# ml4ai/mliis

Hardware: AMD Instinct MI355X
Metric: inner-loop images/sec (EfficientLab-6-3, 224x224, 5-shot) (higher is better)
Workload: dtype f32 (the long-K decoder convs and their filter gradients with every operand split exactly into three bf16 terms on the matrix cores, 6 term products, f32 accumulate: fp32-equivalent products; everything else the fp32 instruction)

## Files before the change

mliis_amd/csrc/dwmarch.hip:

```cpp
#include "bn_fold.hpp"
#include "common.hpp"

namespace mliis {

constexpr int kDwmStoreAux = 2;
typedef unsigned dwm_u32x4 __attribute__((ext_vector_type(4)));
constexpr unsigned kDwmOob = 0xFFFFFFF0u;

__device__ __forceinline__ __amdgpu_buffer_rsrc_t dwm_rsrc(const void* p) {
  const unsigned long long u = (unsigned long long)p;
  const unsigned lo = __builtin_amdgcn_readfirstlane((unsigned)u), hi = __builtin_amdgcn_readfirstlane((unsigned)(u >> 32));
  return __builtin_amdgcn_make_buffer_rsrc((void*)(((unsigned long long)hi << 32) | lo), 0, 0x80000000u, 0x00020000);
}

typedef unsigned dwm_u32x2 __attribute__((ext_vector_type(2)));
template <typename T = float>
__device__ __forceinline__ float4 dwm_load(__amdgpu_buffer_rsrc_t r, int off, bool ok) {
  if constexpr (sizeof(T) == 4) {
    const dwm_u32x4 u = __builtin_amdgcn_raw_buffer_load_b128(r, ok ? off : (int)kDwmOob, 0, 0);
    return make_float4(__uint_as_float(u.x), __uint_as_float(u.y), __uint_as_float(u.z), __uint_as_float(u.w));
  } else {
    const dwm_u32x2 u = __builtin_amdgcn_raw_buffer_load_b64(r, ok ? off : (int)kDwmOob, 0, 0);
    return unpack_bf16x4(make_uint2(u.x, u.y));
  }
}

template <typename T = float>
__device__ __forceinline__ void dwm_store(__amdgpu_buffer_rsrc_t r, int off, bool ok, const float4 v) {
  if constexpr (sizeof(T) == 2) {
    const uint2 pk = pack_bf16x4(v);
    dwm_u32x2 u2;
    u2.x = pk.x; u2.y = pk.y;
    __builtin_amdgcn_raw_buffer_store_b64(u2, r, ok ? off : (int)kDwmOob, 0, kDwmStoreAux);
    return;
  }
  dwm_u32x4 u;
  u.x = __float_as_uint(v.x); u.y = __float_as_uint(v.y); u.z = __float_as_uint(v.z); u.w = __float_as_uint(v.w);
  __builtin_amdgcn_raw_buffer_store_b128(u, r, ok ? off : (int)kDwmOob, 0, kDwmStoreAux);
}
__device__ __forceinline__ float4 f4sel(bool ok, const float4 v) { return ok ? v : make_float4(0.f, 0.f, 0.f, 0.f); }
template <typename T> __device__ __forceinline__ float4 dwm_stored(const float4 v) { return stored_value(static_cast<const T*>(nullptr), v); }

template <int K, int S>
struct MarchCfg {
  static constexpr int TS = S == 1 ? 4 : 2;
  static constexpr int BW = 7 * TS;
  static constexpr int SPR = BW / TS;
  static constexpr int RS = 4;
  static constexpr int IBW = (BW - 1) * S + K;
  static constexpr int IBWP = (IBW + 1) & ~1;
  static constexpr int WIN = (RS - 1) * S + K;
  static constexpr int NEW = RS * S;
  static constexpr int NR = WIN + NEW;
  static constexpr int WW = (TS - 1) * S + K;
  static_assert(IBW <= 32, "one pixel lane per ring column");
  static_assert(WIN <= 2 * NEW, "head batch + batch 0 cover the window of step 0");
};

struct DwmBn {
  BnFold f;
  const float* gamma;
  const float* beta;
};

struct DwmDyBn {
  const float* z;
  const float *mean, *rstd, *gamma, *beta;
  const float *gate, *chan_add;
  const float* stage1;
  int nimg;
  double inv_rows;
  float *dgamma, *dbeta;
};
struct DwmDyQuad {
  float4 sc, sh, gt, ca, k1, k0;
};
__device__ __forceinline__ DwmDyQuad dwm_dybn_setup(const DwmDyBn& d, int C, int c0, int q, bool cok, int n, bool lead) {
  const int c = cok ? c0 + q * 4 : 0;
  const float4 m = ld4(d.mean + c), rs = ld4(d.rstd + c), ga = ld4(d.gamma + c), be = ld4(d.beta + c);
  DwmDyQuad k;
  k.gt = ld4(d.gate + (long long)n * C + c);
  k.ca = ld4(d.chan_add + (long long)n * C + c);
  double s1[4] = {0, 0, 0, 0}, s2[4] = {0, 0, 0, 0};
  for (int i0 = 0; i0 < d.nimg; i0 += 8) {
    float4 u[8], v[8];
#pragma unroll
    for (int j = 0; j < 8; ++j) {
      const int i = i0 + j < d.nimg ? i0 + j : d.nimg - 1;
      u[j] = ld4(d.stage1 + ((long long)i * 2 + 0) * C + c);
      v[j] = ld4(d.stage1 + ((long long)i * 2 + 1) * C + c);
    }
#pragma unroll
    for (int j = 0; j < 8; ++j)
      if (i0 + j < d.nimg) {
        s1[0] += u[j].x; s1[1] += u[j].y; s1[2] += u[j].z; s1[3] += u[j].w;
        s2[0] += v[j].x; s2[1] += v[j].y; s2[2] += v[j].z; s2[3] += v[j].w;
      }
  }
  if (lead && cok && (threadIdx.x >> 3) == 0) {
    st4(d.dbeta + c, make_float4((float)s1[0], (float)s1[1], (float)s1[2], (float)s1[3]));
    st4(d.dgamma + c, make_float4((float)s2[0], (float)s2[1], (float)s2[2], (float)s2[3]));
  }
  const float4 a = make_float4((float)(s1[0] * d.inv_rows), (float)(s1[1] * d.inv_rows), (float)(s1[2] * d.inv_rows), (float)(s1[3] * d.inv_rows));
  const float4 b = make_float4((float)(s2[0] * d.inv_rows), (float)(s2[1] * d.inv_rows), (float)(s2[2] * d.inv_rows), (float)(s2[3] * d.inv_rows));
  k.sc = f4mul(ga, rs);
  k.sh = make_float4(fmaf(-m.x, k.sc.x, be.x), fmaf(-m.y, k.sc.y, be.y), fmaf(-m.z, k.sc.z, be.z), fmaf(-m.w, k.sc.w, be.w));
  k.k1 = make_float4(-k.sc.x * b.x * rs.x, -k.sc.y * b.y * rs.y, -k.sc.z * b.z * rs.z, -k.sc.w * b.w * rs.w);
  k.k0 = make_float4(-k.sc.x * a.x - k.k1.x * m.x, -k.sc.y * a.y - k.k1.y * m.y, -k.sc.z * a.z - k.k1.z * m.z, -k.sc.w * a.w - k.k1.w * m.w);
  return k;
}
__device__ __forceinline__ float dwm_dz1(float da2, float z, float sc, float sh, float gt, float ca, float k1, float k0) {
  const float u = fmaf(z, sc, sh);
  const float sg = sigmoid_f(u);
  const float g = fmaf(da2, gt, ca) * (sg * (1.0f + u * (1.0f - sg)));
  return fmaf(sc, g, fmaf(z, k1, k0));
}
__device__ __forceinline__ float4 dwm_dz1(const float4 da2, const float4 z, const DwmDyQuad& k) {
  return make_float4(dwm_dz1(da2.x, z.x, k.sc.x, k.sh.x, k.gt.x, k.ca.x, k.k1.x, k.k0.x), dwm_dz1(da2.y, z.y, k.sc.y, k.sh.y, k.gt.y, k.ca.y, k.k1.y, k.k0.y),
                     dwm_dz1(da2.z, z.z, k.sc.z, k.sh.z, k.gt.z, k.ca.z, k.k1.z, k.k0.z), dwm_dz1(da2.w, z.w, k.sc.w, k.sh.w, k.gt.w, k.ca.w, k.k1.w, k.k0.w));
}

template <int NEW, bool TWO>
struct DwmBatch {
  float4 a[NEW];
  float4 b[TWO ? NEW : 1];
};

struct DwmArgs {
  const float* x;
  const float* w;
  float* y;
  int Hi, Wi, Ho, Wo;
  int C, pt, pl;
  int bands, bw, chunks, rpc;
  float* stats_part;
  DwmBn bn;
  DwmDyBn dyb;
  const float* z;
  float* dw_part;
};

struct DwmQuad {
  float4 sc, sh, m, rs;
};

__device__ __forceinline__ float4 dwm_act(const float4 z, const DwmQuad& k) {
  float4 u = make_float4(fmaf(z.x, k.sc.x, k.sh.x), fmaf(z.y, k.sc.y, k.sh.y), fmaf(z.z, k.sc.z, k.sh.z), fmaf(z.w, k.sc.w, k.sh.w));
  return make_float4(swish_f(u.x), swish_f(u.y), swish_f(u.z), swish_f(u.w));
}

constexpr int kDwmFoldBatch = 8;
template <bool FOLD>
struct DwmBnState {
  float4 g, b, m, rs;
  FoldAcc acc;
  float4 u[FOLD ? kDwmFoldBatch : 1], v[FOLD ? kDwmFoldBatch : 1];
  int k;
};
template <bool FOLD>
__device__ __forceinline__ void dwm_bn_begin(const DwmBn& bn, int C, int c0, int q, bool cok, DwmBnState<FOLD>& st) {
  const int c = cok ? c0 + q * 4 : 0;
  st.g = ld4(bn.gamma + c);
  st.b = ld4(bn.beta + c);
  if (FOLD && bn.f.nblk > 0) {
    const int bl = threadIdx.x >> 3;
    st.k = bl;
    for (; st.k + 32 * kDwmFoldBatch < bn.f.nblk; st.k += 32 * kDwmFoldBatch) {
      fold_issue<FOLD ? kDwmFoldBatch : 1>(bn.f.part, bn.f.nblk, C, c, st.k, bl, st.u, st.v);
      if (cok) fold_add<FOLD ? kDwmFoldBatch : 1>(st.acc, bn.f.nblk, st.k, st.u, st.v);
    }
    fold_issue<FOLD ? kDwmFoldBatch : 1>(bn.f.part, bn.f.nblk, C, c, st.k, st.k < bn.f.nblk ? st.k : 0, st.u, st.v);
  } else {
    st.m = ld4(bn.f.mean + c);
    st.rs = ld4(bn.f.rstd + c);
  }
}
template <bool FOLD>
__device__ __forceinline__ DwmQuad dwm_bn_end(const DwmBn& bn, int C, int c0, int q, bool cok, bool lead, double* smd, float* s_mr ,
                                              DwmBnState<FOLD>& st) {
  const int t = threadIdx.x;
  DwmQuad k;
  if (FOLD && bn.f.nblk > 0) {
    if (cok) fold_add<FOLD ? kDwmFoldBatch : 1>(st.acc, bn.f.nblk, st.k, st.u, st.v);
    double s, ss;
    fold_finish(st.acc, smd, s, ss);
    if (t < 32) {
      const double m = s * bn.f.inv_n;
      double var = ss * bn.f.inv_n - m * m;
      if (var < 0.0) var = 0.0;
      const float mf = (float)m, rf = (float)(1.0 / sqrt(var + (double)bn.f.eps));
      s_mr[t] = mf;
      s_mr[32 + t] = rf;
      const int cc = c0 + t;
      if (lead && cc < C) {
        bn.f.mean[cc] = mf;
        bn.f.rstd[cc] = rf;
        if (bn.f.moving_mean != nullptr) {
          const float mm = bn.f.moving_mean[cc], mv = bn.f.moving_var[cc];
          bn.f.moving_mean[cc] = mm - (mm - mf) * bn.f.one_minus_momentum;
          bn.f.moving_var[cc] = mv - (mv - (float)(var * (double)bn.f.ema_var_factor)) * bn.f.one_minus_momentum;
        }
      }
    }
    __syncthreads();
    k.m = ld4(s_mr + q * 4);
    k.rs = ld4(s_mr + 32 + q * 4);
    __syncthreads();
  } else {
    k.m = st.m;
    k.rs = st.rs;
  }
  k.sc = f4mul(st.g, k.rs);
  k.sh = make_float4(fmaf(-k.m.x, k.sc.x, st.b.x), fmaf(-k.m.y, k.sc.y, st.b.y), fmaf(-k.m.z, k.sc.z, st.b.z), fmaf(-k.m.w, k.sc.w, st.b.w));
  return k;
}

__device__ __forceinline__ void dwm_emit_pair(const float4 s1, const float4 s2, float4* buf, float* __restrict__ part, unsigned blk, int C,
                                              int c0) {
  const int t = threadIdx.x;
  buf[t] = s1;
  buf[256 + t] = s2;
  __syncthreads();
  float4 v = f4zero();
  if (t < 64) {
    const int qq = t & 7, g = (t >> 3) & 3, vv = t >> 5;
#pragma unroll
    for (int i = 0; i < 8; ++i) v = f4add(v, buf[vv * 256 + (g * 8 + i) * 8 + qq]);
  }
  __syncthreads();
  if (t < 64) buf[t] = v;
  __syncthreads();
  if (t < 16) {
    const int qq = t & 7, vv = t >> 3;
    const int cc = c0 + qq * 4;
    const float4* b4 = buf + vv * 32 + qq;
    if (cc < C) st4(part + ((long long)blk * 2 + vv) * C + cc, f4add(f4add(b4[0], b4[8]), f4add(b4[16], b4[24])));
  }
}

template <int K, int S, bool PRE, bool BWD, bool DYBN = false, typename TA = float, typename TB = float>
__global__ __launch_bounds__(256, BWD ? 1 : 2) void dwm_conv_k(const DwmArgs a) {
  constexpr int EA = (int)sizeof(TA), EB = (int)sizeof(TB);
  static_assert(!DYBN || BWD, "DYBN is a backward mode");
  typedef MarchCfg<K, S> G;
  constexpr int TS = G::TS, SPR = G::SPR, RS = G::RS, IBW = G::IBW, IBWP = G::IBWP, WIN = G::WIN, NEW = G::NEW, NR = G::NR, WW = G::WW;
  static_assert(!BWD || S == 1, "the stride-2 backward is dwm_bwd_s2_k");
  constexpr int kRingF4 = (NR * IBWP + 1) * 8;
  constexpr int kTrash = NR * IBWP * 8;
  constexpr int kScratchF4 = BWD ? (K * K * 4 * 8) : 0;
  constexpr int kSharedF4 = kRingF4 > kScratchF4 ? kRingF4 : kScratchF4;
  static_assert(kSharedF4 * 16 >= 2 * 32 * 32 * 8, "the statistics fold borrows the ring");
  __shared__ float4 ring[kSharedF4];
  __shared__ float4 wl[K * K * 8];
  __shared__ __attribute__((aligned(16))) float s_mr[64];

  const int t = threadIdx.x, q = t & 7, p = t >> 3;
  const unsigned bx = xcd_remap(blockIdx.x, gridDim.x);
  const int chunk = (int)(bx % (unsigned)a.chunks);
  const unsigned r_ = bx / (unsigned)a.chunks;
  const int band = (int)(r_ % (unsigned)a.bands), n = (int)(r_ / (unsigned)a.bands);
  const int c0 = blockIdx.y * 32, c = c0 + q * 4;
  const bool cok = c < a.C;
  const int Hi = a.Hi, Wi = a.Wi, Ho = a.Ho, Wo = a.Wo, C = a.C;
  const int oy0 = chunk * a.rpc;
  const int oy1 = oy0 + a.rpc < Ho ? oy0 + a.rpc : Ho;
  const int ox0 = band * a.bw;
  const int bwa = a.bw < Wo - ox0 ? a.bw : Wo - ox0;
  const int iy0 = oy0 * S - a.pt, ix0 = ox0 * S - a.pl;
  const int ibw = (bwa - 1) * S + K;
  const int rows_needed = (oy1 - oy0 - 1) * S + K;
  const int nsteps = (oy1 - oy0 + RS - 1) / RS;
  const __amdgpu_buffer_rsrc_t rX = dwm_rsrc(a.x);
  const __amdgpu_buffer_rsrc_t rZ = dwm_rsrc((BWD ? a.z : a.x));
  const __amdgpu_buffer_rsrc_t rY = dwm_rsrc(a.y);

  const bool colok = cok && p < ibw && (unsigned)(ix0 + p) < (unsigned)Wi;
  const int tbase = (((n * Hi + iy0) * Wi + ix0 + p) * C + c) * EA;
  const int rowbytes = Wi * C * EA;
  const int lcol = p < IBWP ? (p ^ ((p >> 2) & 1)) * 8 + q : kTrash + q;
  auto row_in = [&](int rr) { return rr >= 0 && rr < rows_needed && (unsigned)(iy0 + rr) < (unsigned)Hi; };
  typedef DwmBatch<NEW, DYBN> Batch;
  const __amdgpu_buffer_rsrc_t rX2 = dwm_rsrc(DYBN ? a.dyb.z : a.x);
  auto issue = [&](Batch& r, int rb) {
#pragma unroll
    for (int j = 0; j < NEW; ++j) {
      r.a[j] = dwm_load<TA>(rX, tbase + (rb + j) * rowbytes, colok && row_in(rb + j));
      if (DYBN) r.b[j] = dwm_load<TA>(rX2, tbase + (rb + j) * rowbytes, colok && row_in(rb + j));
    }
  };
  DwmQuad kq;
  DwmDyQuad dq;
  auto commit = [&](const Batch& r, int rb, int sb) {
#pragma unroll
    for (int j = 0; j < NEW; ++j) {
      float4 v = r.a[j];
      if (PRE && !BWD) v = f4sel(colok && row_in(rb + j), dwm_act(v, kq));
      if (DYBN) v = f4sel(colok && row_in(rb + j), dwm_dz1(v, r.b[j], dq));
      int slot = sb + j;
      if (slot >= NR) slot -= NR;
      if (rb + j >= 0) ring[(p < IBWP ? slot * (IBWP * 8) : 0) + lcol] = v;
    }
  };

  const int ro = p >> 3, sx = p & 7;
  const bool item_ok = sx < SPR && cok;
  const int colbase = sx < SPR ? sx * (TS * S) : 0;
  const int sxpar = sx & 1;
  const int zbase = BWD ? (((n * Ho + oy0 + ro) * Wo + ox0 + sx * TS) * C + c) * EB : 0;
  auto issue_z = [&](float4 (&zr)[TS], int step) {
    if (BWD) {
      const int oy = oy0 + step * RS + ro;
      const int base = zbase + step * RS * Wo * C * EB;
#pragma unroll
      for (int u = 0; u < TS; ++u) zr[u] = dwm_load<TB>(rZ, base + u * C * EB, item_ok && oy < oy1 && sx * TS + u < bwa);
    }
  };

  constexpr int HEAD = WIN - 2 * NEW;
  float4 wreg = f4zero();
  if (t < K * K * 8) {
    const int tap = t >> 3, qq = t & 7;
    const int cc = c0 + qq * 4;
    if (cc < C) wreg = ld4(a.w + (long long)(BWD ? K * K - 1 - tap : tap) * C + cc);
  }
  DwmBnState<!BWD> bst;
  if (PRE) dwm_bn_begin(a.bn, C, c0, q, cok, bst);
  if (DYBN) dq = dwm_dybn_setup(a.dyb, C, c0, q, cok, n, bx == 0);
  Batch ra, rb_;
  float4 za[TS], zb[TS];
  {
    Batch h0, h1;
    issue(h0, HEAD);
    issue(h1, WIN - NEW);
    issue_z(za, 0);
    if (PRE) kq = dwm_bn_end(a.bn, C, c0, q, cok, bx == 0, reinterpret_cast<double*>(ring), s_mr, bst);
    issue(ra, WIN);
    issue(rb_, WIN + NEW);
    issue_z(zb, 1);
    if (t < K * K * 8) wl[t] = wreg;
    commit(h0, HEAD, HEAD < 0 ? HEAD + NR : HEAD);
    commit(h1, WIN - NEW, (WIN - NEW) % NR);
  }
  __syncthreads();

  float4 s1 = f4zero(), s2 = f4zero();
  float4 dwacc[BWD ? K * K : 1];
  if (BWD) {
#pragma unroll
    for (int k = 0; k < K * K; ++k) dwacc[k] = f4zero();
  }

  int sw = 0;
  auto compute = [&](int step, const float4 (&zr)[TS]) {
    const int oy = oy0 + step * RS + ro;
    const bool row_ok = item_ok && oy < oy1;
    int s0 = sw + ro * S;
    if (s0 >= NR) s0 -= NR;
    float4 acc[TS];
#pragma unroll
    for (int u = 0; u < TS; ++u) acc[u] = f4zero();
    int wofs = q;
    if (K == 5) asm volatile("" : "+v"(wofs));
    const float4* wq = wl + wofs;
    float4 av[TS], sgm[TS];
    if (BWD) {
#pragma unroll
      for (int u = 0; u < TS; ++u) {
        const bool ok = row_ok && sx * TS + u < bwa;
        if (PRE) {
          const float4 z = zr[u];
          const float4 uu = make_float4(fmaf(z.x, kq.sc.x, kq.sh.x), fmaf(z.y, kq.sc.y, kq.sh.y), fmaf(z.z, kq.sc.z, kq.sh.z), fmaf(z.w, kq.sc.w, kq.sh.w));
          sgm[u] = f4sel(ok, make_float4(sigmoid_f(uu.x), sigmoid_f(uu.y), sigmoid_f(uu.z), sigmoid_f(uu.w)));
          av[u] = f4mul(uu, sgm[u]);
        } else {
          av[u] = f4sel(ok, zr[u]);
        }
      }
    }
    auto read_row = [&](int ky, float4 (&in)[WW]) {
      int slot = s0 + ky;
      if (slot >= NR) slot -= NR;
      if constexpr ((TS * S) % 4 == 0) {
        const float4* rowp = ring + slot * (IBWP * 8) + colbase * 8 + q;
        const float4* A0 = rowp + sxpar * 8;
        const float4* A1 = rowp - sxpar * 8;
#pragma unroll
        for (int j = 0; j < WW; ++j) {
          const int je = j ^ ((j >> 2) & 1);
          in[j] = ((je & 1) ? A1 : A0)[je * 8];
        }
      } else {
        const float4* rowp = ring + slot * (IBWP * 8) + q;
#pragma unroll
        for (int j = 0; j < WW; ++j) {
          const int col = colbase + j;
          in[j] = rowp[(col ^ ((col >> 2) & 1)) * 8];
        }
      }
    };
    auto fma_row = [&](int ky, const float4 (&in)[WW]) {
      float4 wk[K];
#pragma unroll
      for (int kx = 0; kx < K; ++kx) wk[kx] = wq[(ky * K + kx) * 8];
#pragma unroll
      for (int kx = 0; kx < K; ++kx)
#pragma unroll
        for (int u = 0; u < TS; ++u) {
          acc[u] = f4fma(in[u * S + kx], wk[kx], acc[u]);
          if (BWD) dwacc[ky * K + kx] = f4fma(in[u + kx], av[u], dwacc[ky * K + kx]);
        }
    };
    if (K == 3) {
      float4 in[WW];
#pragma unroll
      for (int ky = 0; ky < K; ++ky) {
        read_row(ky, in);
        fma_row(ky, in);
      }
    } else {
      float4 inA[WW], inB[WW];
      read_row(0, inA);
#pragma unroll
      for (int ky = 0; ky < K; ++ky) {
        if (ky + 1 < K) read_row(ky + 1, (ky & 1) ? inA : inB);
        fma_row(ky, (ky & 1) ? inB : inA);
        __builtin_amdgcn_sched_barrier(0);
      }
    }
    const int ybase = (((n * Ho + oy) * Wo + ox0 + sx * TS) * C + c) * EB;
    if (K == 5 && EB == 2) __builtin_amdgcn_sched_barrier(0);
#pragma unroll
    for (int u = 0; u < TS; ++u) {
      const bool ok = row_ok && sx * TS + u < bwa;
      if (!(K == 5 && !BWD)) acc[u] = dwm_stored<TB>(acc[u]);
      dwm_store<TB>(rY, ybase + u * C * EB, ok, acc[u]);
      if (!BWD) {
        const float4 v = f4sel(ok, acc[u]);
        s1 = f4add(s1, v);
        s2 = f4fma(v, v, s2);
      } else if (PRE) {
        const float4 z = zr[u], sg_ = sgm[u];
        const float4 uu = make_float4(fmaf(z.x, kq.sc.x, kq.sh.x), fmaf(z.y, kq.sc.y, kq.sh.y), fmaf(z.z, kq.sc.z, kq.sh.z), fmaf(z.w, kq.sc.w, kq.sh.w));
        const float4 g = make_float4(acc[u].x * sg_.x * (1.0f + uu.x * (1.0f - sg_.x)), acc[u].y * sg_.y * (1.0f + uu.y * (1.0f - sg_.y)),
                                     acc[u].z * sg_.z * (1.0f + uu.z * (1.0f - sg_.z)), acc[u].w * sg_.w * (1.0f + uu.w * (1.0f - sg_.w)));
        const float4 xh = make_float4((z.x - kq.m.x) * kq.rs.x, (z.y - kq.m.y) * kq.rs.y, (z.z - kq.m.z) * kq.rs.z, (z.w - kq.m.w) * kq.rs.w);
        s1 = f4add(s1, g);
        s2 = f4fma(g, xh, s2);
      }
    }
  };

  int rbn = WIN;
  int sbn = WIN % NR;
  for (int i = 0; i < nsteps; i += 2) {
    compute(i, za);
    commit(ra, rbn, sbn);
    issue(ra, rbn + 2 * NEW);
    issue_z(za, i + 2);
    rbn += NEW; sbn += NEW; if (sbn >= NR) sbn -= NR;
    sw += NEW; if (sw >= NR) sw -= NR;
    __syncthreads();
    if (i + 1 < nsteps) compute(i + 1, zb);
    commit(rb_, rbn, sbn);
    issue(rb_, rbn + 2 * NEW);
    issue_z(zb, i + 3);
    rbn += NEW; sbn += NEW; if (sbn >= NR) sbn -= NR;
    sw += NEW; if (sw >= NR) sw -= NR;
    __syncthreads();
  }

  if (a.stats_part != nullptr && (!BWD || PRE)) dwm_emit_pair(s1, s2, ring, a.stats_part, bx, C, c0);
  if (BWD) {
    __syncthreads();
    float4* fold = ring;
#pragma unroll
    for (int k = 0; k < K * K; ++k) {
      float4 v = dwacc[k];
#pragma unroll
      for (int off = 8; off < 64; off <<= 1) {
        v.x += __shfl_xor(v.x, off); v.y += __shfl_xor(v.y, off); v.z += __shfl_xor(v.z, off); v.w += __shfl_xor(v.w, off);
      }
      if ((t & 63) < 8) fold[(k * 4 + (t >> 6)) * 8 + q] = v;
    }
    __syncthreads();
    for (int e = t; e < K * K * 8; e += 256) {
      const int k = e >> 3, qq = e & 7;
      const int cc = c0 + qq * 4;
      if (cc < C)
        st4(a.dw_part + ((long long)bx * (K * K) + (K * K - 1 - k)) * C + cc,
            f4add(f4add(fold[(k * 4 + 0) * 8 + qq], fold[(k * 4 + 1) * 8 + qq]), f4add(fold[(k * 4 + 2) * 8 + qq], fold[(k * 4 + 3) * 8 + qq])));
    }
  }
}

template <int K, bool PRE, bool DYBN = false, typename TA = float, typename TB = float>
__global__ __launch_bounds__(256, (K == 5 || DYBN) ? 1 : 2) void dwm_bwd_s2_k(const DwmArgs a) {
  constexpr int EA = (int)sizeof(TA), EB = (int)sizeof(TB);
  constexpr int BP = 14;
  constexpr int D = (K - 1) / 2;
  constexpr int NEWD = 2, WIND = 2 + D, NR = WIND + NEWD, IBW = 16;
  static_assert(BP + D <= IBW, "one pixel lane per ring pixel of a batch");
  constexpr int kRingF4 = NR * IBW * 8;
  constexpr int kScratchF4 = K * K * 4 * 8;
  constexpr int kSharedF4 = (kRingF4 > kScratchF4 ? kRingF4 : kScratchF4) > 1024 ? (kRingF4 > kScratchF4 ? kRingF4 : kScratchF4) : 1024;
  __shared__ float4 ring[kSharedF4];
  __shared__ float4 wl[K * K * 8];
  __shared__ __attribute__((aligned(16))) float s_mr[64];

  const int t = threadIdx.x, q = t & 7, p = t >> 3;
  const unsigned bx = xcd_remap(blockIdx.x, gridDim.x);
  const int chunk = (int)(bx % (unsigned)a.chunks);
  const unsigned r_ = bx / (unsigned)a.chunks;
  const int band = (int)(r_ % (unsigned)a.bands), n = (int)(r_ / (unsigned)a.bands);
  const int c0 = blockIdx.y * 32, c = c0 + q * 4;
  const bool cok = c < a.C;
  const int Hd = a.Hi, Wd = a.Wi, H = a.Ho, W = a.Wo, C = a.C, pt = a.pt, pl = a.pl;
  const int my_lo = pt >> 1, my_hi = (H + pt - 1) >> 1;
  const int mx_lo = pl >> 1, mx_hi = (W + pl - 1) >> 1;
  const int m0 = my_lo + chunk * a.rpc;
  const int m1 = m0 + a.rpc <= my_hi + 1 ? m0 + a.rpc : my_hi + 1;
  const int x0 = mx_lo + band * a.bw;
  const int bpa = a.bw < mx_hi + 1 - x0 ? a.bw : mx_hi + 1 - x0;
  const int nsteps = (m1 - m0 + 1) / 2;
  const int rows_needed = m1 - m0 + D;
  const __amdgpu_buffer_rsrc_t rX = dwm_rsrc(a.x);
  const __amdgpu_buffer_rsrc_t rZ = dwm_rsrc(a.z);
  const __amdgpu_buffer_rsrc_t rY = dwm_rsrc(a.y);

  const int sl = p >> 4, scol = p & 15;
  const bool colok = cok && scol < bpa + D && (unsigned)(x0 - D + scol) < (unsigned)Wd;
  const int tbase = (((n * Hd + m0 - D + sl) * Wd + x0 - D + scol) * C + c) * EA;
  const int rowbytes = Wd * C * EA;
  typedef DwmBatch<1, DYBN> Batch;
  const __amdgpu_buffer_rsrc_t rX2 = dwm_rsrc(DYBN ? a.dyb.z : a.x);
  auto row_in = [&](int rr) { return rr >= 0 && rr < rows_needed && (unsigned)(m0 - D + rr) < (unsigned)Hd; };
  auto issue = [&](Batch& r, int rb) {
    r.a[0] = dwm_load<TA>(rX, tbase + rb * rowbytes, colok && row_in(rb + sl));
    if (DYBN) r.b[0] = dwm_load<TA>(rX2, tbase + rb * rowbytes, colok && row_in(rb + sl));
  };
  DwmDyQuad dq;
  auto commit = [&](const Batch& r, int rb, int sb) {
    int slot = sb + sl;
    if (slot >= NR) slot -= NR;
    float4 v = r.a[0];
    if (DYBN) v = f4sel(colok && row_in(rb + sl), dwm_dz1(v, r.b[0], dq));
    if (rb + sl >= 0) ring[slot * (IBW * 8) + scol * 8 + q] = v;
  };

  const int rp = p >> 4, px = p & 15;
  const bool item_ok = px < bpa && cok;
  const int pxc = px < BP ? px : 0;
  const int wi0 = 2 * (x0 + px) - pl;
  auto pix_ok = [&](int step, int u) {
    const int hi = 2 * (m0 + 2 * step + rp) + (u >> 1) - pt, wi = wi0 + (u & 1);
    return item_ok && m0 + 2 * step + rp < m1 && (unsigned)hi < (unsigned)H && (unsigned)wi < (unsigned)W;
  };
  auto pix_off = [&](int step, int u) {
    const int hi = 2 * (m0 + 2 * step + rp) + (u >> 1) - pt, wi = wi0 + (u & 1);
    return (((n * H + hi) * W + wi) * C + c) * EB;
  };
  auto issue_z = [&](float4 (&zr)[4], int step) {
#pragma unroll
    for (int u = 0; u < 4; ++u) zr[u] = dwm_load<TB>(rZ, pix_off(step, u), pix_ok(step, u));
  };

  constexpr int HEAD = WIND - 2 * NEWD;
  float4 wreg = f4zero();
  if (t < K * K * 8) {
    const int tap = t >> 3, qq = t & 7;
    const int cc = c0 + qq * 4;
    if (cc < C) wreg = ld4(a.w + (long long)tap * C + cc);
  }
  DwmQuad kq;
  DwmBnState<false> bst;
  if (PRE) dwm_bn_begin(a.bn, C, c0, q, cok, bst);
  if (PRE) kq = dwm_bn_end(a.bn, C, c0, q, cok, false, reinterpret_cast<double*>(ring), s_mr, bst);
  if (DYBN) dq = dwm_dybn_setup(a.dyb, C, c0, q, cok, n, bx == 0);
  Batch ra, rb_, h0, h1;
  float4 za[4], zb[4];
  issue(h0, HEAD);
  issue(h1, WIND - NEWD);
  issue_z(za, 0);
  issue(ra, WIND);
  issue(rb_, WIND + NEWD);
  issue_z(zb, 1);
  if (t < K * K * 8) wl[t] = wreg;
  commit(h0, HEAD, HEAD < 0 ? HEAD + NR : HEAD);
  commit(h1, WIND - NEWD, (WIND - NEWD) % NR);
  __syncthreads();

  float4 s1 = f4zero(), s2 = f4zero();
  float4 dwacc[K * K];
#pragma unroll
  for (int k = 0; k < K * K; ++k) dwacc[k] = f4zero();

  int sw = 0;
  auto compute = [&](int step, const float4 (&zr)[4]) {
    float4 av[4], sgm[4], acc[4];
#pragma unroll
    for (int u = 0; u < 4; ++u) {
      const bool ok = pix_ok(step, u);
      acc[u] = f4zero();
      if (PRE) {
        const float4 z = zr[u];
        const float4 uu = make_float4(fmaf(z.x, kq.sc.x, kq.sh.x), fmaf(z.y, kq.sc.y, kq.sh.y), fmaf(z.z, kq.sc.z, kq.sh.z), fmaf(z.w, kq.sc.w, kq.sh.w));
        sgm[u] = f4sel(ok, make_float4(sigmoid_f(uu.x), sigmoid_f(uu.y), sigmoid_f(uu.z), sigmoid_f(uu.w)));
        av[u] = f4mul(uu, sgm[u]);
      } else {
        av[u] = f4sel(ok, zr[u]);
      }
    }
    int s0 = sw + rp;
    if (s0 >= NR) s0 -= NR;
    int wofs = q;
    if (K == 5) asm volatile("" : "+v"(wofs));
    const float4* wq = wl + wofs;
#pragma unroll
    for (int wr = 0; wr <= D; ++wr) {
      int slot = s0 + wr;
      if (slot >= NR) slot -= NR;
      const float4* rowp = ring + slot * (IBW * 8) + pxc * 8 + q;
      float4 dv[D + 1];
#pragma unroll
      for (int wc = 0; wc <= D; ++wc) dv[wc] = rowp[wc * 8];
#pragma unroll
      for (int pa = 0; pa < 2; ++pa) {
        const int ky = pa + 2 * (D - wr);
        if (ky > K - 1) continue;
#pragma unroll
        for (int wc = 0; wc <= D; ++wc)
#pragma unroll
          for (int pb = 0; pb < 2; ++pb) {
            const int kx = pb + 2 * (D - wc);
            if (kx > K - 1) continue;
            const int u = pa * 2 + pb, tap = ky * K + kx;
            acc[u] = f4fma(dv[wc], wq[tap * 8], acc[u]);
            dwacc[tap] = f4fma(dv[wc], av[u], dwacc[tap]);
          }
      }
      __builtin_amdgcn_sched_barrier(0);
    }
#pragma unroll
    for (int u = 0; u < 4; ++u) {
      acc[u] = dwm_stored<TB>(acc[u]);
      dwm_store<TB>(rY, pix_off(step, u), pix_ok(step, u), acc[u]);
      if (PRE) {
        const float4 z = zr[u], sg_ = sgm[u];
        const float4 uu = make_float4(fmaf(z.x, kq.sc.x, kq.sh.x), fmaf(z.y, kq.sc.y, kq.sh.y), fmaf(z.z, kq.sc.z, kq.sh.z), fmaf(z.w, kq.sc.w, kq.sh.w));
        const float4 g = make_float4(acc[u].x * sg_.x * (1.0f + uu.x * (1.0f - sg_.x)), acc[u].y * sg_.y * (1.0f + uu.y * (1.0f - sg_.y)),
                                     acc[u].z * sg_.z * (1.0f + uu.z * (1.0f - sg_.z)), acc[u].w * sg_.w * (1.0f + uu.w * (1.0f - sg_.w)));
        const float4 xh = make_float4((z.x - kq.m.x) * kq.rs.x, (z.y - kq.m.y) * kq.rs.y, (z.z - kq.m.z) * kq.rs.z, (z.w - kq.m.w) * kq.rs.w);
        s1 = f4add(s1, g);
        s2 = f4fma(g, xh, s2);
      }
    }
  };

  int rbn = WIND, sbn = WIND % NR;
  for (int i = 0; i < nsteps; i += 2) {
    compute(i, za);
    commit(ra, rbn, sbn);
    issue(ra, rbn + 2 * NEWD);
    issue_z(za, i + 2);
    rbn += NEWD; sbn += NEWD; if (sbn >= NR) sbn -= NR;
    sw += NEWD; if (sw >= NR) sw -= NR;
    __syncthreads();
    if (i + 1 < nsteps) compute(i + 1, zb);
    commit(rb_, rbn, sbn);
    issue(rb_, rbn + 2 * NEWD);
    issue_z(zb, i + 3);
    rbn += NEWD; sbn += NEWD; if (sbn >= NR) sbn -= NR;
    sw += NEWD; if (sw >= NR) sw -= NR;
    __syncthreads();
  }

  if (a.stats_part != nullptr && PRE) dwm_emit_pair(s1, s2, ring, a.stats_part, bx, C, c0);
  __syncthreads();
  float4* fold = ring;
#pragma unroll
  for (int k = 0; k < K * K; ++k) {
    float4 v = dwacc[k];
#pragma unroll
    for (int off = 8; off < 64; off <<= 1) {
      v.x += __shfl_xor(v.x, off); v.y += __shfl_xor(v.y, off); v.z += __shfl_xor(v.z, off); v.w += __shfl_xor(v.w, off);
    }
    if ((t & 63) < 8) fold[(k * 4 + (t >> 6)) * 8 + q] = v;
  }
  __syncthreads();
  for (int e = t; e < K * K * 8; e += 256) {
    const int k = e >> 3, qq = e & 7;
    const int cc = c0 + qq * 4;
    if (cc < C)
      st4(a.dw_part + ((long long)bx * (K * K) + k) * C + cc,
          f4add(f4add(fold[(k * 4 + 0) * 8 + qq], fold[(k * 4 + 1) * 8 + qq]), f4add(fold[(k * 4 + 2) * 8 + qq], fold[(k * 4 + 3) * 8 + qq])));
  }
}

struct MarchGeom {
  int bands, bw, chunks, rpc;
  int Ho, Wo, pt, pl;
  long long gx;
  int gy;
};

static inline void same_pad(int H, int K, int S, int* Ho, int* pt) {
  *Ho = (H + S - 1) / S;
  int th = (*Ho - 1) * S + K - H;
  if (th < 0) th = 0;
  *pt = th / 2;
}

static int g_dwm_target = -1;
static inline int dwm_target(bool bwd) {
  if (g_dwm_target < 0) {
    const char* e = getenv("MLIIS_DWM_TARGET");
    g_dwm_target = e ? atoi(e) : 0;
    if (g_dwm_target < 0) g_dwm_target = 0;
  }
  return g_dwm_target ? g_dwm_target : (bwd ? 256 : 448);
}

static inline void march_split(int N, int cgs, int P, int Q, int unit, int bmax, int ts, bool bwd, MarchGeom* g) {
  g->bands = (Q + bmax - 1) / bmax;
  int bw = (Q + g->bands - 1) / g->bands;
  bw = (bw + ts - 1) / ts * ts;
  g->bw = bw;
  g->bands = (Q + bw - 1) / bw;
  const long long base = (long long)N * cgs * g->bands;
  long long chunks = dwm_target(bwd) / base;
  const int max_chunks = (P + 2 * unit - 1) / (2 * unit);
  if (chunks > max_chunks) chunks = max_chunks;
  if (chunks < 1) chunks = 1;
  int rpc = (int)((P + chunks - 1) / chunks);
  rpc = (rpc + unit - 1) / unit * unit;
  g->rpc = rpc;
  g->chunks = (P + rpc - 1) / rpc;
  g->gx = (long long)N * g->bands * g->chunks;
  g->gy = cgs;
}

static inline MarchGeom march_geom_fwd(int N, int H, int W, int C, int K, int S) {
  MarchGeom g;
  same_pad(H, K, S, &g.Ho, &g.pt);
  same_pad(W, K, S, &g.Wo, &g.pl);
  if (S == 1) march_split(N, ceil_div(C, 32), g.Ho, g.Wo, 4, 28, 4, false, &g);
  else march_split(N, ceil_div(C, 32), g.Ho, g.Wo, 4, 14, 2, false, &g);
  return g;
}

static inline MarchGeom march_geom_bwd(int N, int H, int W, int C, int K, int S) {
  MarchGeom g;
  same_pad(H, K, S, &g.Ho, &g.pt);
  same_pad(W, K, S, &g.Wo, &g.pl);
  if (S == 1) {
    march_split(N, ceil_div(C, 32), H, W, 4, 28, 4, true, &g);
  } else {
    const int py = ((H + g.pt - 1) >> 1) - (g.pt >> 1) + 1, pxn = ((W + g.pl - 1) >> 1) - (g.pl >> 1) + 1;
    march_split(N, ceil_div(C, 32), py, pxn, 2, 14, 1, true, &g);
  }
  return g;
}

static inline DwmBn make_bn(const float* part, int nblk, long long count, const float* gamma, const float* beta, float* mean, float* rstd,
                            float* moving_mean, float* moving_var, float eps, float momentum, int unbiased) {
  DwmBn b;
  b.f.part = part;
  b.f.nblk = nblk;
  b.f.inv_n = 1.0 / (double)count;
  b.f.eps = eps;
  b.f.one_minus_momentum = 1.0f - momentum;
  b.f.ema_var_factor = (unbiased && count > 1) ? (float)((double)count / (double)(count - 1)) : 1.0f;
  b.f.mean = mean;
  b.f.rstd = rstd;
  b.f.moving_mean = moving_mean;
  b.f.moving_var = moving_var;
  b.gamma = gamma;
  b.beta = beta;
  return b;
}

static inline bool dwm_types_ok(bool bwd, int ta, int tb) {
  if (ta == MLIIS_DT_F32 && tb == MLIIS_DT_F32) return true;
  if (ta == MLIIS_DT_BF16 && tb == MLIIS_DT_BF16) return true;
  return bwd ? (ta == MLIIS_DT_BF16 && tb == MLIIS_DT_F32) : (ta == MLIIS_DT_F32 && tb == MLIIS_DT_BF16);
}
template <int K, int S, bool PRE, bool BWD>
static void launch_conv(const MarchGeom& g, const DwmArgs& a, int ta, int tb, hipStream_t stream) {
  const dim3 grid((unsigned)g.gx, g.gy);
  if (ta == MLIIS_DT_F32 && tb == MLIIS_DT_F32) hipLaunchKernelGGL((dwm_conv_k<K, S, PRE, BWD, false, float, float>), grid, dim3(256), 0, stream, a);
  else if (ta == MLIIS_DT_BF16 && tb == MLIIS_DT_BF16) hipLaunchKernelGGL((dwm_conv_k<K, S, PRE, BWD, false, bf16s, bf16s>), grid, dim3(256), 0, stream, a);
  else if constexpr (BWD) hipLaunchKernelGGL((dwm_conv_k<K, S, PRE, BWD, false, bf16s, float>), grid, dim3(256), 0, stream, a);
  else hipLaunchKernelGGL((dwm_conv_k<K, S, PRE, BWD, false, float, bf16s>), grid, dim3(256), 0, stream, a);
}
template <int K, bool PRE>
static void launch_bwd_s2(const MarchGeom& g, const DwmArgs& a, int ta, int tb, hipStream_t stream) {
  const dim3 grid((unsigned)g.gx, g.gy);
  if (ta == MLIIS_DT_F32) hipLaunchKernelGGL((dwm_bwd_s2_k<K, PRE, false, float, float>), grid, dim3(256), 0, stream, a);
  else if (tb == MLIIS_DT_BF16) hipLaunchKernelGGL((dwm_bwd_s2_k<K, PRE, false, bf16s, bf16s>), grid, dim3(256), 0, stream, a);
  else hipLaunchKernelGGL((dwm_bwd_s2_k<K, PRE, false, bf16s, float>), grid, dim3(256), 0, stream, a);
}
template <int K, typename TA, typename TB>
static void launch_bwd_dybn_t(const MarchGeom& g, const DwmArgs& a, int stride, hipStream_t stream) {
  const dim3 grid((unsigned)g.gx, g.gy);
  if (stride == 1) hipLaunchKernelGGL((dwm_conv_k<K, 1, true, true, true, TA, TB>), grid, dim3(256), 0, stream, a);
  else hipLaunchKernelGGL((dwm_bwd_s2_k<K, true, true, TA, TB>), grid, dim3(256), 0, stream, a);
}
template <int K>
static void launch_bwd_dybn(const MarchGeom& g, const DwmArgs& a, int stride, int ta, int tb, hipStream_t stream) {
  if (ta == MLIIS_DT_F32) launch_bwd_dybn_t<K, float, float>(g, a, stride, stream);
  else if (tb == MLIIS_DT_BF16) launch_bwd_dybn_t<K, bf16s, bf16s>(g, a, stride, stream);
  else launch_bwd_dybn_t<K, bf16s, float>(g, a, stride, stream);
}

}

using namespace mliis;

static int dwm_check(const char* name, int N, int H, int W, int C, int k, int stride) {
  MLIIS_REQUIRE(N > 0 && H > 0 && W > 0 && C > 0 && (C & 3) == 0, MLIIS_ERR_ARG, "%s: bad shape N=%d H=%d W=%d C=%d (C %% 4 must be 0)", name, N, H,
                W, C);
  MLIIS_REQUIRE((k == 3 || k == 5) && (stride == 1 || stride == 2), MLIIS_ERR_UNSUPPORTED, "%s: unsupported k=%d stride=%d", name, k, stride);
  MLIIS_REQUIRE((long long)N * H * W * C * 4 < (1LL << 31), MLIIS_ERR_UNSUPPORTED, "%s: tensor larger than 2 GiB (32-bit buffer offsets)", name);
  return MLIIS_OK;
}

extern "C" {

int mliis_dwconv_bn_supported(int N, int H, int W, int C, int k, int stride) {
  if (N <= 0 || H <= 0 || W <= 0 || C <= 0 || (C & 3) || (k != 3 && k != 5) || (stride != 1 && stride != 2)) return 0;
  return ((long long)N * H * W * C * 4 < (1LL << 31)) ? 1 : 0;
}

int mliis_dwconv_bn_fwd_blocks(int N, int H, int W, int C, int k, int stride) {
  if (N <= 0 || H <= 0 || W <= 0 || C <= 0 || (C & 3) || (k != 3 && k != 5) || (stride != 1 && stride != 2)) return 0;
  return (int)march_geom_fwd(N, H, W, C, k, stride).gx;
}

int mliis_dwconv_bn_bwd_blocks(int N, int H, int W, int C, int k, int stride) {
  if (N <= 0 || H <= 0 || W <= 0 || C <= 0 || (C & 3) || (k != 3 && k != 5) || (stride != 1 && stride != 2)) return 0;
  return (int)march_geom_bwd(N, H, W, C, k, stride).gx;
}

int mliis_dwconv_bn_fwd(const float* z, const float* bn_part, int bn_nblk, const float* bn_gamma, const float* bn_beta, float* bn_mean,
                        float* bn_rstd, float* bn_moving_mean, float* bn_moving_var, float eps, float momentum, const float* w, float* y,
                        int N, int H, int W, int C, int k, int stride, float* stats_part, size_t stats_floats, int* stats_nblk,
                        int in_dtype, int out_dtype, hipStream_t stream) {
  int rc = dwm_check("dwconv_bn_fwd", N, H, W, C, k, stride);
  if (rc) return rc;
  MLIIS_REQUIRE(dwm_types_ok(false, in_dtype, out_dtype), MLIIS_ERR_ARG, "dwconv_bn_fwd: unsupported storage types (in %d, out %d)", in_dtype, out_dtype);
  MLIIS_REQUIRE(z && w && y && aligned16(z) && aligned16(w) && aligned16(y), MLIIS_ERR_ARG, "dwconv_bn_fwd: null or unaligned pointer");
  const bool pre = bn_gamma != nullptr;
  if (pre) {
    MLIIS_REQUIRE(bn_beta && bn_mean && bn_rstd && aligned16(bn_gamma) && aligned16(bn_beta), MLIIS_ERR_ARG,
                  "dwconv_bn_fwd: the batch norm needs gamma, beta (16-byte aligned) and mean / rstd vectors");
    MLIIS_REQUIRE(bn_nblk >= 0 && (bn_nblk == 0 || (bn_part && aligned16(bn_part))), MLIIS_ERR_ARG, "dwconv_bn_fwd: bad statistics partials");
    MLIIS_REQUIRE((bn_moving_mean == nullptr) == (bn_moving_var == nullptr), MLIIS_ERR_ARG, "dwconv_bn_fwd: moving mean / variance come as a pair");
  }
  const MarchGeom g = march_geom_fwd(N, H, W, C, k, stride);
  MLIIS_REQUIRE(g.gx < (1LL << 31), MLIIS_ERR_UNSUPPORTED, "dwconv_bn_fwd: too many workgroups");
  if (stats_nblk) *stats_nblk = 0;
  if (stats_part != nullptr) {
    MLIIS_REQUIRE(stats_nblk && aligned16(stats_part), MLIIS_ERR_ARG, "dwconv_bn_fwd: statistics need a 16-byte aligned buffer and a stats_nblk output");
    MLIIS_REQUIRE((size_t)g.gx * 2 * C <= stats_floats, MLIIS_ERR_WORKSPACE, "dwconv_bn_fwd: statistics buffer too small (%zu floats needed, %zu given)",
                  (size_t)g.gx * 2 * C, stats_floats);
    *stats_nblk = (int)g.gx;
  }
  DwmArgs a{};
  a.x = z; a.w = w; a.y = y;
  a.Hi = H; a.Wi = W; a.Ho = g.Ho; a.Wo = g.Wo; a.C = C; a.pt = g.pt; a.pl = g.pl;
  a.bands = g.bands; a.bw = g.bw; a.chunks = g.chunks; a.rpc = g.rpc;
  a.stats_part = stats_part;
  if (pre) a.bn = make_bn(bn_part, bn_nblk, (long long)N * H * W, bn_gamma, bn_beta, bn_mean, bn_rstd, bn_moving_mean, bn_moving_var, eps, momentum, 0);
#define DWM_FWD(K_, S_)                                             \
  do {                                                              \
    if (pre) launch_conv<K_, S_, true, false>(g, a, in_dtype, out_dtype, stream);  \
    else launch_conv<K_, S_, false, false>(g, a, in_dtype, out_dtype, stream);     \
  } while (0)
  if (k == 3 && stride == 1) DWM_FWD(3, 1);
  else if (k == 3) DWM_FWD(3, 2);
  else if (stride == 1) DWM_FWD(5, 1);
  else DWM_FWD(5, 2);
#undef DWM_FWD
  MLIIS_CHECK_LAUNCH("dwconv_bn_fwd");
  return MLIIS_OK;
}

int mliis_dwconv_bn_bwd(const float* dy, const float* z, const float* bn_mean, const float* bn_rstd, const float* bn_gamma,
                        const float* bn_beta, const float* w, float* dx, float* dw, int N, int H, int W, int C, int k, int stride,
                        float* dw_part, size_t dw_part_floats, float* bn_part, size_t bn_part_floats, int* nblk, int dy_dtype, int zx_dtype,
                        hipStream_t stream) {
  int rc = dwm_check("dwconv_bn_bwd", N, H, W, C, k, stride);
  if (rc) return rc;
  MLIIS_REQUIRE(dwm_types_ok(true, dy_dtype, zx_dtype), MLIIS_ERR_ARG, "dwconv_bn_bwd: unsupported storage types (dy %d, z / dx %d)", dy_dtype, zx_dtype);
  MLIIS_REQUIRE(dy && z && w && dx && dw_part && nblk && aligned16(dy) && aligned16(z) && aligned16(w) && aligned16(dx) && aligned16(dw_part),
                MLIIS_ERR_ARG, "dwconv_bn_bwd: null or unaligned pointer");
  const bool pre = bn_gamma != nullptr;
  if (pre)
    MLIIS_REQUIRE(bn_beta && bn_mean && bn_rstd && aligned16(bn_gamma) && aligned16(bn_beta) && (bn_part == nullptr || aligned16(bn_part)),
                  MLIIS_ERR_ARG, "dwconv_bn_bwd: the batch norm needs gamma, beta (16-byte aligned), mean and rstd");
  const MarchGeom g = march_geom_bwd(N, H, W, C, k, stride);
  MLIIS_REQUIRE(g.gx < (1LL << 31), MLIIS_ERR_UNSUPPORTED, "dwconv_bn_bwd: too many workgroups");
  MLIIS_REQUIRE((size_t)g.gx * k * k * C <= dw_part_floats, MLIIS_ERR_WORKSPACE, "dwconv_bn_bwd: filter-gradient slabs need %zu floats, %zu given",
                (size_t)g.gx * k * k * C, dw_part_floats);
  MLIIS_REQUIRE(!pre || bn_part == nullptr || (size_t)g.gx * 2 * C <= bn_part_floats, MLIIS_ERR_WORKSPACE,
                "dwconv_bn_bwd: batch-norm partials need %zu floats, %zu given", (size_t)g.gx * 2 * C, bn_part_floats);
  *nblk = (int)g.gx;
  DwmArgs a{};
  a.x = dy; a.w = w; a.y = dx; a.z = z;
  a.C = C;
  a.bands = g.bands; a.bw = g.bw; a.chunks = g.chunks; a.rpc = g.rpc;
  a.stats_part = pre ? bn_part : nullptr;
  a.dw_part = dw_part;
  if (pre) a.bn = make_bn(nullptr, 0, 1, bn_gamma, bn_beta, const_cast<float*>(bn_mean), const_cast<float*>(bn_rstd), nullptr, nullptr, 0.f, 0.f, 0);
  if (stride == 1) {
    a.Hi = H; a.Wi = W; a.Ho = H; a.Wo = W; a.pt = k - 1 - g.pt; a.pl = k - 1 - g.pl;
    if (k == 3) { if (pre) launch_conv<3, 1, true, true>(g, a, dy_dtype, zx_dtype, stream); else launch_conv<3, 1, false, true>(g, a, dy_dtype, zx_dtype, stream); }
    else { if (pre) launch_conv<5, 1, true, true>(g, a, dy_dtype, zx_dtype, stream); else launch_conv<5, 1, false, true>(g, a, dy_dtype, zx_dtype, stream); }
  } else {
    a.Hi = g.Ho; a.Wi = g.Wo; a.Ho = H; a.Wo = W; a.pt = g.pt; a.pl = g.pl;
    if (k == 3) { if (pre) launch_bwd_s2<3, true>(g, a, dy_dtype, zx_dtype, stream); else launch_bwd_s2<3, false>(g, a, dy_dtype, zx_dtype, stream); }
    else { if (pre) launch_bwd_s2<5, true>(g, a, dy_dtype, zx_dtype, stream); else launch_bwd_s2<5, false>(g, a, dy_dtype, zx_dtype, stream); }
  }
  MLIIS_CHECK_LAUNCH("dwconv_bn_bwd");
  if (dw != nullptr) {
    MLIIS_REQUIRE(aligned16(dw), MLIIS_ERR_ALIGN, "dwconv_bn_bwd: dw must be 16-byte aligned");
    hipLaunchKernelGGL(fold_flat_k, dim3(ceil_div(k * k * C, kFoldX)), dim3(kFoldX, kFoldY), 0, stream, dw_part, (int)g.gx, (long long)k * k * C, 1.0f,
                       dw, 0, (long long)k * k * C, 0LL, 0LL);
    MLIIS_CHECK_LAUNCH("dwconv_bn_bwd_fold");
  }
  return MLIIS_OK;
}

int mliis_mbconv_dw_bwd_march(const float* da2, const float* z1, const float* mean1, const float* rstd1, const float* gamma1, const float* beta1,
                              const float* gate, const float* chan_add, const float* stage1, int stage1_nimg, float* dgamma1, float* dbeta1,
                              const float* z0, const float* mean0, const float* rstd0, const float* gamma0, const float* beta0, const float* w,
                              float* dx, int N, int H, int W, int C, int k, int stride, float* dw_part, size_t dw_part_floats, float* bn_part,
                              size_t bn_part_floats, int* nblk, int dy_dtype, int zx_dtype, hipStream_t stream) {
  int rc = dwm_check("mbconv_dw_bwd_march", N, H, W, C, k, stride);
  if (rc) return rc;
  MLIIS_REQUIRE(dwm_types_ok(true, dy_dtype, zx_dtype), MLIIS_ERR_ARG, "mbconv_dw_bwd_march: unsupported storage types (da2 / z1 %d, z0 / dx %d)", dy_dtype, zx_dtype);
  MLIIS_REQUIRE(da2 && z1 && mean1 && rstd1 && gamma1 && beta1 && gate && chan_add && stage1 && stage1_nimg > 0 && dgamma1 && dbeta1 && z0 && mean0 &&
                    rstd0 && gamma0 && beta0 && w && dx && dw_part && bn_part && nblk,
                MLIIS_ERR_ARG, "mbconv_dw_bwd_march: null pointer");
  MLIIS_REQUIRE(aligned16(da2) && aligned16(z1) && aligned16(mean1) && aligned16(rstd1) && aligned16(gamma1) && aligned16(beta1) && aligned16(gate) &&
                    aligned16(chan_add) && aligned16(stage1) && aligned16(dgamma1) && aligned16(dbeta1) && aligned16(z0) && aligned16(mean0) &&
                    aligned16(rstd0) && aligned16(gamma0) && aligned16(beta0) && aligned16(w) && aligned16(dx) && aligned16(dw_part) && aligned16(bn_part),
                MLIIS_ERR_ALIGN, "mbconv_dw_bwd_march: pointers must be 16-byte aligned");
  const MarchGeom g = march_geom_bwd(N, H, W, C, k, stride);
  MLIIS_REQUIRE(g.gx < (1LL << 31), MLIIS_ERR_UNSUPPORTED, "mbconv_dw_bwd_march: too many workgroups");
  MLIIS_REQUIRE((size_t)g.gx * k * k * C <= dw_part_floats && (size_t)g.gx * 2 * C <= bn_part_floats, MLIIS_ERR_WORKSPACE,
                "mbconv_dw_bwd_march: slab buffers too small (%zu / %zu floats needed)", (size_t)g.gx * k * k * C, (size_t)g.gx * 2 * C);
  *nblk = (int)g.gx;
  DwmArgs a{};
  a.x = da2; a.w = w; a.y = dx; a.z = z0;
  a.C = C;
  a.bands = g.bands; a.bw = g.bw; a.chunks = g.chunks; a.rpc = g.rpc;
  a.stats_part = bn_part;
  a.dw_part = dw_part;
  a.bn = make_bn(nullptr, 0, 1, gamma0, beta0, const_cast<float*>(mean0), const_cast<float*>(rstd0), nullptr, nullptr, 0.f, 0.f, 0);
  a.dyb = DwmDyBn{z1, mean1, rstd1, gamma1, beta1, gate, chan_add, stage1, stage1_nimg, 1.0 / ((double)N * g.Ho * g.Wo), dgamma1, dbeta1};
  if (stride == 1) {
    a.Hi = H; a.Wi = W; a.Ho = H; a.Wo = W; a.pt = k - 1 - g.pt; a.pl = k - 1 - g.pl;
  } else {
    a.Hi = g.Ho; a.Wi = g.Wo; a.Ho = H; a.Wo = W; a.pt = g.pt; a.pl = g.pl;
  }
  if (k == 3) launch_bwd_dybn<3>(g, a, stride, dy_dtype, zx_dtype, stream);
  else launch_bwd_dybn<5>(g, a, stride, dy_dtype, zx_dtype, stream);
  MLIIS_CHECK_LAUNCH("mbconv_dw_bwd_march");
  return MLIIS_OK;
}
}
```

mliis_amd/passes.py:

```python
from __future__ import annotations

import torch

from . import ops, spec
from ._lib import MliisError
from .plan import _Plan


class _Pass:

    def __init__(self, L, P: _Plan, training: bool, stochastic: bool = True):
        self.L, self.P, self.training = L, P, training
        self.stochastic = training and stochastic
        self.w, self.mv, self.g, self.ws = L.arena.w, L.arena.mv, L.arena.g, L.ws

    def moving(self, prefix):
        return self.mv[prefix + "/moving_mean"], self.mv[prefix + "/moving_variance"]

    def bn_bwd_args(self, st, prefix):
        return st[0], st[1], self.w[prefix + "/gamma"], self.w[prefix + "/beta"]

    def bn_fwd_args(self, st, prefix, moving=True):
        return (self.w[prefix + "/gamma"], self.w[prefix + "/beta"], st[0], st[1]) + (self.moving(prefix) if moving else (None, None))

    def moving_stats(self, st, prefix):
        mean, var = self.moving(prefix)
        st[0].copy_(mean)
        torch.rsqrt(var + spec.BN_EPS, out=st[1])

    def bn(self, xin, st, prefix, y, pre=False, post=False, img_scale=None, res=None, fused=False, nblk=0, pool_part=None, always_batch=False,
           part=None):
        P = self.P
        if self.training or always_batch:
            part = P.stats_part if (part is None or nblk == 0) else part
            if nblk == 0:
                nblk = ops.bn_stats_partial(xin, pre, P.stats_part)
            return ops.bn_apply_fused(xin, part, nblk, *self.bn_bwd_args(st, prefix), moving=self.moving(prefix) if self.training else None,
                                      unbiased_moving_var=fused, pre_swish=pre, post_swish=post, img_scale=img_scale, res=res, out=y,
                                      pool_part=pool_part)
        self.moving_stats(st, prefix)
        return ops.bn_apply(xin, *self.bn_bwd_args(st, prefix), pre, post, img_scale, res, out=y)

    def bn_in(self, z, st, prefix, nblk):
        if self.training:
            if nblk == 0:
                nblk = ops.bn_stats_partial(z, False, self.P.stats_part)
            return self.bn_fwd_args(st, prefix), nblk
        self.moving_stats(st, prefix)
        return self.bn_fwd_args(st, prefix, moving=False), 0

    def conv(self, xin, wname, bname, dil, out, swish_stats, x_scale=None, border_bias=None, out_block=0, part=None, bnin=None):
        L, P, w = self.L, self.P, self.w
        am = L._amax_of.get(wname)
        if bnin is not None:
            return ops.conv2d_fwd_bnin(bnin["z"], P.stats_part3, bnin["nblk"], *self.bn_bwd_args(bnin["st"], bnin["prefix"]), xin, w[wname], out,
                                       moving=self.moving(bnin["prefix"]), img_scale=bnin["img_scale"], res=bnin["res"], stats_part=P.stats_part,
                                       stats_swish=swish_stats, wt=L.wt[wname], precision=L.matmul_precision, fp8_w_amax=am, out_block=out_block)[1]
        part = (P.stats_part if part is None else part) if self.training else None
        bias, swish_stats = (w[bname] if bname else None), bool(swish_stats and self.training)
        if L._x3_takes(wname, xin):
            r = ops.conv2d_fwd_x3(xin, L.x3.image(wname, "fwd"), w[wname].shape[0], w[wname].shape[3], bias, dil, out=out, ws=self.ws,
                                  stats_part=part, stats_swish=swish_stats, border_bias=border_bias)
        else:
            r = L._conv_fwd(xin, w[wname], bias, dil, out=out, ws=self.ws, stats_part=part, stats_swish=swish_stats, wt=L.wt[wname],
                            x_scale=x_scale, border_bias=border_bias, fp8_w_amax=am, out_block=out_block)
        return r[1] if self.training else 0

    def dwconv(self, xin, wname, stride, out):
        if self.training:
            return ops.dwconv_fwd(xin, self.w[wname], stride, out=out, stats_part=self.P.stats_part)[1]
        ops.dwconv_fwd(xin, self.w[wname], stride, out=out)
        return 0

    def bn_b(self, xin, dy, st, prefix, dx, pre=False, post=False, img_scale=None, chan_scale=None, chan_add=None, dskip=None,
             dskip_accumulate=False, dxsum_part=None, stage1=None):
        ops.bn_bwd(xin, dy, *self.bn_bwd_args(st, prefix), pre, post, img_scale, chan_scale, chan_add, dx=dx, dgamma=self.g[prefix + "/gamma"],
                   dbeta=self.g[prefix + "/beta"], ws=self.ws, dskip=dskip, dskip_accumulate=dskip_accumulate, dxsum_part=dxsum_part, stage1=stage1)

    def wgrad_conv(self, xin, dz, kk, dil, key, x_scale=None):
        P = self.P
        if not P.wbatch_ready:
            P.wbatch.add(xin, dz, kk, dil, P.fold_part[key], x_scale=x_scale)

    def conv_bwd_data(self, dz, wname, dil, cin, out, accumulate=False):
        L = self.L
        if L._x3_takes(wname, dz):
            ops.conv2d_bwd_data_x3(dz, L.x3.image(wname, "bwd"), 3, cin, dil, out=out, accumulate=accumulate, ws=self.ws)
        else:
            L._conv_bwd_data(dz, self.w[wname], dil, ci_begin=0, ci_count=cin, out=out, accumulate=accumulate, ws=self.ws)

    def noexpand_dw_bwd(self, B, tgt, tgt_has, dw_bwd_data):
        if tgt_has:
            dw_bwd_data(B["da0"])
            ops.chan_affine(B["da0"], out=tgt, accumulate=True)
        else:
            dw_bwd_data(tgt)


class _Passes:
    X3_MIN_ROWS = 8192

    def _x3_takes(self, wname, xin) -> bool:
        return self.x3 is not None and self.x3.has(wname, "fwd") and xin.shape[0] * xin.shape[1] * xin.shape[2] >= self.X3_MIN_ROWS

    def _forward(self, P: _Plan, x, idx, training: bool, upsample: bool = True, stochastic: bool = True):
        a, S = self.arch, _Pass(self, P, training, stochastic)
        ops.transpose_weights(self.arena.theta, self.theta_t, self.wt_desc, self.w_amax, tiles=self.wt_tiles, x3=self.x3, rng=self._rng_now)
        self._rng_now = None
        cur, nb_stem = self._stem_fwd(S, x, idx)
        pend = None
        for bi, (b, B, nm) in enumerate(zip(a.executed(), P.blocks, self.n_blocks)):
            B["x_in"] = cur
            if training and B["small"]:
                cur, pend = self._mbconv_small_fwd(S, bi, b, B, nm, cur, pend)
            elif B["march"]:
                cur, pend = self._mbconv_march_fwd(S, bi, b, B, nm, cur, pend, nb_stem)
            else:
                cur, pend = self._mbconv_opbyop_fwd(S, bi, b, B, nm, cur, pend)
        if pend is not None:
            raise MliisError("internal: a deferred project batch norm was not consumed")
        ends = {r: P.blocks[bi]["out"] for r, bi in a.reductions.items() if bi < len(P.blocks)}
        dec = ends[4]
        if a.aspp:
            dec = self._aspp_forward(P, dec, S.stochastic)
        if a.skipdec is not None:
            dec = self._skipdec_fwd(S, dec, ends)
        for j in range(len(a.rsd)):
            dec = self._rsd_fwd(S, j, dec, ends)
        mask = P.drop_mask if (S.stochastic and P.drop_mask is not None) else None
        P.dec_in = dec
        ops.final_conv_fwd(dec, S.w[self.n_final[0]], S.w[self.n_final[1]], mask, out=P.small)
        H = a.image_size
        if not upsample:
            return None
        ops.resize_bilinear_fwd(P.small, (H, H), out=P.logits)
        return P.logits

    def _stem_fwd(self, S: _Pass, x, idx):
        P, w = S.P, S.w
        nb = 0
        if S.training:
            nb = max(0, ops.stem_conv_fwd(x, w[self.n_stem[0]], idx, out=P.z_stem, stats_part=P.stats_part)[1])
        else:
            ops.stem_conv_fwd(x, w[self.n_stem[0]], idx, out=P.z_stem)
        if P.fuse_stem:
            return None, nb
        return S.bn(P.z_stem, P.st_stem, self.n_stem[1], P.a_stem, post=True, nblk=nb), 0

    def _mbconv_small_fwd(self, S: _Pass, bi, b, B, nm, x, bnin):
        P, w = S.P, S.w
        z0 = B["z0b"] if B["blk"] else B["z0"]
        nb = S.conv(x, nm["w_exp"], None, 1, z0, False, out_block=B["blk"], bnin=bnin)
        if nb == 0:
            if B["blk"]:
                raise MliisError("internal: the streamed expand conv of block {} left no statistics".format(b.idx))
            nb = ops.bn_stats_partial(z0, False, P.stats_part)
        ops.mbconv_dw_fwd_small(z0, P.stats_part, nb, S.bn_fwd_args(B["st0"], nm["bn0"]), w[nm["w_dw"]], S.bn_fwd_args(B["st1"], nm["bn1"]),
                                B["z1"], B["a1"], B["s"], z0_blocked=B["z0b"], z1_blocked=True)
        return self._mbconv_tail_fwd(S, bi, b, B, nm)

    def _mbconv_march_fwd(self, S: _Pass, bi, b, B, nm, x, bnin, nb_stem):
        P, w = S.P, S.w
        if b.expand != 1:
            nb = S.conv(x, nm["w_exp"], None, 1, B["z0"], False, bnin=bnin)
            bn0, nb = S.bn_in(B["z0"], B["st0"], nm["bn0"], nb)
            zin = B["z0"]
        elif bi == 0 and P.fuse_stem:
            bn0, nb = S.bn_in(P.z_stem, P.st_stem, self.n_stem[1], nb_stem)
            zin = P.z_stem
        else:
            bn0, nb, zin = None, 0, x
        if S.training:
            nb = ops.dwconv_bn_fwd(zin, w[nm["w_dw"]], b.stride, bn=bn0, part=P.stats_part, nblk=nb, out=B["z1"], stats_part=P.stats_part2)[1]
        else:
            ops.dwconv_bn_fwd(zin, w[nm["w_dw"]], b.stride, bn=bn0, out=B["z1"])
            nb = 0
        return self._mbconv_bn1_fwd(S, bi, b, B, nm, nb, P.stats_part2)

    def _mbconv_opbyop_fwd(self, S: _Pass, bi, b, B, nm, x, bnin):
        if b.expand != 1:
            nb = S.conv(x, nm["w_exp"], None, 1, B["z0"], False, bnin=bnin)
            x = S.bn(B["z0"], B["st0"], nm["bn0"], B["a0"], post=True, nblk=nb)
        nb = S.dwconv(x, nm["w_dw"], b.stride, B["z1"])
        return self._mbconv_bn1_fwd(S, bi, b, B, nm, nb, S.P.stats_part)

    def _mbconv_bn1_fwd(self, S: _Pass, bi, b, B, nm, nb, st_part):
        P = S.P
        if S.training:
            chunks = S.bn(B["z1"], B["st1"], nm["bn1"], B["a1"], post=True, nblk=nb, pool_part=P.pool_part, part=st_part)[1]
            return self._mbconv_tail_fwd(S, bi, b, B, nm, pool_chunks=chunks)
        S.bn(B["z1"], B["st1"], nm["bn1"], B["a1"], post=True, nblk=nb)
        ops.colsum(B["a1"], None, nseg=P.N, scale=1.0 / (b.h_out * b.h_out), out=B["s"], ws=S.ws)
        return self._mbconv_tail_fwd(S, bi, b, B, nm)

    def _mbconv_tail_fwd(self, S: _Pass, bi, b, B, nm, pool_chunks=None):
        P = S.P
        se = [S.w[k] for k in nm["se"]]
        if pool_chunks is None:
            ops.se_mlp_fwd(B["s"], *se, B["hpre"], B["gate"])
        else:
            ops.se_mlp_fwd(P.pool_part, *se, B["hpre"], B["gate"], chunks=pool_chunks, scale=1.0 / (b.h_out * b.h_out), s_out=B["s"])
        defer = S.training and P.bn2_deferred[bi]
        nb = S.conv(B["a1"], nm["w_proj"], None, 1, B["z2"], False, x_scale=B["gate"], part=P.stats_part3 if defer else None)
        use_dc = B["use_dc"] = S.stochastic and self.drop_connect and b.skip and b.drop_rate > 0
        img_scale, res = (B["dc"] if use_dc else None), (B["x_in"] if b.skip else None)
        if defer:
            if nb == 0:
                nb = ops.bn_stats_partial(B["z2"], False, P.stats_part3)
            return B["out"], dict(z=B["z2"], nblk=nb, st=B["st2"], prefix=nm["bn2"], img_scale=img_scale, res=res)
        return S.bn(B["z2"], B["st2"], nm["bn2"], B["out"], img_scale=img_scale, res=res, nblk=nb), None

    def _skipdec_fwd(self, S: _Pass, dec, ends):
        sd, T = self.arch.skipdec, S.P.skipdec
        (k0, n0), seps = self.n_skipdec
        cur = T["cat"]
        ops.resize_bilinear_fwd(dec, (sd.h, sd.h), out=cur[..., :sd.c_in])
        nb = S.conv(ends[2], k0, None, 1, T["z0"], False)
        S.bn(T["z0"], T["st0"], n0, cur[..., sd.c_in:], post=True, fused=True, nblk=nb, always_batch=True)
        for Q, (dwn, dbn, pwn, pbn) in zip(T["sep"], seps):
            Q["x_in"] = cur
            nb = S.dwconv(cur, dwn, 1, Q["zd"])
            S.bn(Q["zd"], Q["std"], dbn, Q["ad"], post=True, fused=True, nblk=nb, always_batch=True)
            nb = S.conv(Q["ad"], pwn, None, 1, Q["zp"], False)
            cur = S.bn(Q["zp"], Q["stp"], pbn, Q["out"], post=True, fused=True, nblk=nb, always_batch=True)
        return cur

    def _rsd_fwd(self, S: _Pass, j, dec, ends):
        P, w, ws = S.P, S.w, S.ws
        m, D, nm = self.arch.rsd[j], P.rsd[j], self.n_rsd[j]
        skip = ends[m.scope_index + 1]
        cat = D["cat"]
        up = cat[..., :m.c_deep]
        pool_chunks = 0
        if m.c_deep % 4 == 0 and (m.c_cat - m.c_deep) % 4 == 0 and m.h > 1:
            pool_chunks = ops.rsd_concat_pool(dec, skip, cat, D["pool_part"])
        else:
            if m.h_in == m.h:
                ops.chan_affine(dec, out=up)
            else:
                ops.resize_bilinear_fwd(dec, (m.h, m.h), out=up)
            ops.chan_affine(skip, out=cat[..., m.c_deep:])
        res_up = up
        if m.upsample_conv:
            ku, bu, nu = self.n_rsd_up[j]
            nb = S.conv(up, ku, bu, 1, D["zu"], True)
            res_up = S.bn(D["zu"], D["stu"], nu, D["up2"], pre=True, fused=True, nblk=nb)
        pyr = D["pyr"]
        (k0, b0, n0), (k1, b1, n1), (kf, bf, nf) = nm
        if S.training:
            nb0 = S.conv(cat, k0, b0, 1, D["z0"], True)
            nb1 = S.conv(cat, k1, b1, 2, D["z1"], True, part=P.stats_part2)
            ops.bn_apply_fused_pair([(D["z" + i], pt, nb_, *S.bn_bwd_args(D["st" + i], nn), S.moving(nn), out_)
                                     for i, pt, nb_, nn, out_ in (("0", P.stats_part, nb0, n0, pyr[..., :m.c_out]),
                                                                  ("1", P.stats_part2, nb1, n1, pyr[..., m.c_out:2 * m.c_out]))],
                                    pre_swish=True, unbiased_moving_var=True)
        else:
            nb = S.conv(cat, k0, b0, 1, D["z0"], True)
            S.bn(D["z0"], D["st0"], n0, pyr[..., :m.c_out], pre=True, fused=True, nblk=nb)
            nb = S.conv(cat, k1, b1, 2, D["z1"], True)
            S.bn(D["z1"], D["st1"], n1, pyr[..., m.c_out:2 * m.c_out], pre=True, fused=True, nblk=nb)
        if pool_chunks:
            ops.rsd_pool_fwd(D["pool_part"], w[kf], 2 * m.c_out, out=D["bbias"], chunks=pool_chunks, scale=1.0 / (m.h * m.h), pool_out=D["pool"])
        else:
            ops.colsum(cat, None, nseg=P.N, scale=1.0 / (m.h * m.h), out=D["pool"], ws=ws)
            ops.rsd_pool_fwd(D["pool"], w[kf], 2 * m.c_out, out=D["bbias"])
        nb = S.conv(pyr, kf, bf, 1, D["zf"], True, border_bias=D["bbias"])
        return S.bn(D["zf"], D["stf"], nf, D["out"], pre=True, res=res_up, fused=True, nblk=nb)

    def _aspp_forward(self, P: _Plan, x, dropout: bool):
        a, w, ws, T, N = self.arch, self.arena.w, self.ws, P.aspp, P.N
        d, hw = a.aspp_dimension, a.aspp_h * a.aspp_h
        (k0, c0), (k1, c1), (k2, c2), (ko, co) = self.n_aspp
        m = T["masks"] if dropout else [None] * 4
        cat = T["cat"]
        self._conv_fwd(x, w[k0], w[c0], 1, out=T["z0"], ws=ws, wt=self.wt[k0], fp8_w_amax=self._amax_of.get(k0))
        ops.swish_mask_fwd(T["z0"], m[0], out=cat[..., 2 * d:])
        self._conv_fwd(x, w[k1], w[c1], spec.ASPP_DILATION, out=T["z1"], ws=ws, wt=self.wt[k1])
        ops.swish_mask_fwd(T["z1"], m[1], out=cat[..., d:2 * d])
        ops.colsum(x, None, nseg=N, scale=1.0 / hw, out=T["pool"], ws=ws)
        self._conv_fwd(T["pool"].view(N, 1, 1, -1), w[k2], w[c2], 1, out=T["z2"].view(N, 1, 1, d), ws=ws, wt=self.wt[k2],
                       fp8_w_amax=self._amax_of.get(k2))
        ops.swish_mask_fwd(T["z2"], m[2], out=T["b2"], pre_mask=True)
        ops.chan_affine(None, A=T["b2"], out=cat[..., :d])
        self._conv_fwd(cat, w[ko], w[co], 1, out=T["zo"], ws=ws, wt=self.wt[ko], fp8_w_amax=self._amax_of.get(ko))
        ops.swish_mask_fwd(T["zo"], m[3], out=T["out"])
        T["trained"] = dropout
        return T["out"]

    def _aspp_backward(self, P: _Plan, x, dx, dx_has: bool):
        a, A, ws, T, N = self.arch, self.arena, self.ws, P.aspp, P.N
        w, g = A.w, A.g
        d, hw = a.aspp_dimension, a.aspp_h * a.aspp_h
        (k0, c0), (k1, c1), (k2, c2), (ko, co) = self.n_aspp
        m = T["masks"]
        cat, dcat = T["cat"], T["dcat"]
        dzo = ops.swish_mask_bwd(T["dout"], T["zo"], m[3], out=T["dzo"])
        self._conv_bwd_filter(cat, dzo, 1, 1, out=g[ko], ws=ws)
        ops.colsum(dzo, out=g[co], ws=ws)
        self._conv_bwd_data(dzo, w[ko], 1, out=dcat, ws=ws)
        d0 = ops.swish_mask_bwd(dcat[..., 2 * d:], T["z0"], m[0], out=dcat[..., 2 * d:])
        self._conv_bwd_filter(x, d0, 1, 1, out=g[k0], ws=ws)
        ops.colsum(d0, out=g[c0], ws=ws)
        self._conv_bwd_data(d0, w[k0], 1, out=dx, accumulate=dx_has, ws=ws)
        d1 = ops.swish_mask_bwd(dcat[..., d:2 * d], T["z1"], m[1], out=dcat[..., d:2 * d])
        self._conv_bwd_filter(x, d1, 3, spec.ASPP_DILATION, out=g[k1], ws=ws)
        ops.colsum(d1, out=g[c1], ws=ws)
        self._conv_bwd_data(d1, w[k1], spec.ASPP_DILATION, out=dx, accumulate=True, ws=ws)
        ops.colsum(dcat[..., :d], None, nseg=N, out=T["db2"], ws=ws)
        d2 = ops.swish_mask_bwd(T["db2"], T["z2"], m[2], out=T["db2"], pre_mask=True)
        pool4, d24 = T["pool"].view(N, 1, 1, -1), d2.view(N, 1, 1, d)
        self._conv_bwd_filter(pool4, d24, 1, 1, out=g[k2], ws=ws)
        ops.colsum(d2, out=g[c2], ws=ws)
        self._conv_bwd_data(d24, w[k2], 1, out=T["dpool"].view(N, 1, 1, -1), ws=ws)
        ops.axpby(0.0, None, 1.0 / hw, T["dpool"])
        ops.chan_affine(None, A=T["dpool"], out=dx, accumulate=True)

    def _backward(self, P: _Plan, x, idx, head_fused: bool = False):
        a, S = self.arch, _Pass(self, P, True)
        w, g = S.w, S.g
        if not head_fused:
            ops.resize_bilinear_bwd(P.dlogits, (a.h_dec, a.h_dec), out=P.dsmall)
        mask = P.drop_mask
        ops.final_conv_bwd_filter(P.dec_in, P.dsmall, mask, dw=g[self.n_final[0]], db=g[self.n_final[1]], ws=S.ws)
        has_grad = [False] * len(P.blocks)
        dtop, _ = self._deep_grad_target(P, has_grad, len(a.rsd))
        ops.final_conv_bwd_data(P.dsmall, w[self.n_final[0]], a.c_final, mask, out=dtop, fin=P.head_fin if head_fused else None)
        if not P.wbatch_ready:
            P.wbatch = ops.FilterBatch(self.device)
        for j in range(len(a.rsd) - 1, -1, -1):
            self._rsd_bwd(S, j, has_grad)
        if a.skipdec is not None:
            self._skipdec_bwd(S, has_grad)
        if a.aspp:
            bi = a.reductions[4]
            self._aspp_backward(P, P.blocks[bi]["out"], P.blocks[bi]["dout"], has_grad[bi])
            has_grad[bi] = True
        stage1 = None
        ex = a.executed()
        for bi in range(len(P.blocks) - 1, -1, -1):
            b, B, nm = ex[bi], P.blocks[bi], self.n_blocks[bi]
            if not has_grad[bi]:
                raise MliisError("internal: block {} has no upstream gradient".format(bi))
            tgt = P.blocks[bi - 1]["dout"] if bi > 0 else P.dstem
            tgt_has = has_grad[bi - 1] if bi > 0 else False
            if B["small"]:
                stage1 = self._mbconv_small_bwd(S, bi, b, B, nm, tgt, tgt_has, stage1)
            elif B["march"]:
                stage1 = self._mbconv_march_bwd(S, bi, b, B, nm, tgt, tgt_has, stage1)
            else:
                stage1 = self._mbconv_opbyop_bwd(S, bi, b, B, nm, tgt, tgt_has, stage1)
            if bi > 0:
                has_grad[bi - 1] = True
        self._stem_bwd(S, x, idx, stage1)
        P.wbatch_ready = True
        P.wbatch.launch("fp32x3" if self.x3 is not None else self.matmul_precision)
        ops.fold_batched(P.fold_buf, self.arena.grad, P.fold_desc, P.fold_tiles, se_desc=P.se_desc, se_tiles=P.se_tiles)

    def _deep_grad_target(self, P: _Plan, has_grad, j):
        a = self.arch
        if j > 0:
            return P.rsd[j - 1]["dout"], False
        if j == 0 and a.skipdec is not None:
            return P.skipdec["dout"], False
        if a.aspp:
            return P.aspp["dout"], False
        bi = a.reductions[4]
        tgt_has, has_grad[bi] = has_grad[bi], True
        return P.blocks[bi]["dout"], tgt_has

    def _rsd_bwd(self, S: _Pass, j, has_grad):
        a, P, w, g, ws = self.arch, S.P, S.w, S.g, S.ws
        m, D, nm = a.rsd[j], P.rsd[j], self.n_rsd[j]
        (k0, b0, n0), (k1, b1, n1), (kf, bf, nf) = nm
        co = m.c_out
        dO, cat, pyr, dpyr, dcat = D["dout"], D["cat"], D["pyr"], D["dpyr"], D["dcat"]
        S.bn_b(D["zf"], dO, D["stf"], nf, D["dzf"], pre=True)
        ops.rsd_pool_bwd(D["dzf"], D["tot"], D["pool"], w[kf], 2 * co, dw=g[kf], dbias=g[bf], dpool=D["dpool"], ws=ws)
        S.wgrad_conv(pyr, D["dzf"], 3, 1, kf)
        S.conv_bwd_data(D["dzf"], kf, 1, 2 * co, dpyr)
        d0, d1 = dpyr[..., :co], dpyr[..., co:2 * co]
        ops.bn_bwd_pair([(D["z" + i], d_, *S.bn_bwd_args(D["st" + i], nn), d_, g[nn + "/gamma"], g[nn + "/beta"], P.fold_part[bb])
                         for i, d_, nn, bb in (("0", d0, n0, b0), ("1", d1, n1, b1))], pre_swish=True, ws=ws)
        tail = P.filter_tail[j]
        cmain = cat[..., :m.c_cat - tail] if tail else cat

        def wgrad(dz, kname, kk, dil, cmain=cmain, ctail=cat[..., m.c_cat - tail:] if tail else None):
            S.wgrad_conv(cmain, dz, kk, dil, kname)
            if ctail is not None:
                S.wgrad_conv(ctail, dz, kk, dil, kname + "#tail")
        wgrad(d0, k0, 1, 1)
        self._conv_bwd_data(d0, w[k0], 1, out=dcat, ws=ws)
        wgrad(d1, k1, 3, 2)
        S.conv_bwd_data(d1, k1, 2, m.c_cat, dcat, accumulate=True)
        bi_skip = a.reductions[m.scope_index + 1]
        if m.upsample_conv:
            ku, bu, nu = self.n_rsd_up[j]
            S.bn_b(D["zu"], dO, D["stu"], nu, D["dzu"], pre=True, dxsum_part=P.fold_part[bu])
            S.wgrad_conv(cat[..., :m.c_deep], D["dzu"], 1, 1, ku)
            self._conv_bwd_data(D["dzu"], w[ku], 1, out=D["dup"], ws=ws)
            dU = D["dup"]
        else:
            dU = dO
        ops.chan_split(dcat, m.c_deep, dU, True, P.blocks[bi_skip]["dout"], has_grad[bi_skip], A=D["dpool"])
        has_grad[bi_skip] = True
        tgt, tgt_has = self._deep_grad_target(P, has_grad, j)
        if m.h_in == m.h:
            ops.chan_affine(dU, out=tgt, accumulate=tgt_has)
        else:
            ops.resize_bilinear_bwd(dU, (m.h_in, m.h_in), out=tgt, accumulate=tgt_has)

    def _skipdec_bwd(self, S: _Pass, has_grad):
        a, P, w, ws = self.arch, S.P, S.w, S.ws
        sd, T = a.skipdec, P.skipdec
        (k0, n0), seps = self.n_skipdec
        d = T["dout"]
        for Q, (dwn, dbn, pwn, pbn) in zip(reversed(T["sep"]), reversed(seps)):
            S.bn_b(Q["zp"], d, Q["stp"], pbn, d, post=True)
            S.wgrad_conv(Q["ad"], d, 1, 1, pwn)
            self._conv_bwd_data(d, w[pwn], 1, out=Q["dad"], ws=ws)
            S.bn_b(Q["zd"], Q["dad"], Q["std"], dbn, Q["dad"], post=True)
            ops.dwconv_bwd_filter(Q["x_in"], Q["dad"], 3, 1, partial=P.fold_part[dwn])
            ops.dwconv_bwd_data(Q["dad"], w[dwn], 1, (sd.h, sd.h), out=Q["din"])
            d = Q["din"]
        bi2 = a.reductions[2]
        S.bn_b(T["z0"], d[..., sd.c_in:], T["st0"], n0, T["dz0"], post=True)
        S.wgrad_conv(P.blocks[bi2]["out"], T["dz0"], 1, 1, k0)
        self._conv_bwd_data(T["dz0"], w[k0], 1, out=P.blocks[bi2]["dout"], accumulate=has_grad[bi2], ws=ws)
        has_grad[bi2] = True
        tgt, tgt_has = self._deep_grad_target(P, has_grad, -1)
        ops.resize_bilinear_bwd(d[..., :sd.c_in], (sd.h_in, sd.h_in), out=tgt, accumulate=tgt_has)

    def _mbconv_project_bwd(self, S: _Pass, b, B, nm, tgt, tgt_has, stage1, out_block=0, bn1_sums=True):
        P, w, ws, N = S.P, S.w, S.ws, S.P.N
        dout, da2, hw = B["dout"], B["da2"], b.h_out * b.h_out
        S.bn_b(B["z2"], dout, B["st2"], nm["bn2"], dout, img_scale=B["dc"] if B["use_dc"] else None,
               dskip=tgt if b.skip else None, dskip_accumulate=tgt_has, stage1=stage1)
        S.wgrad_conv(B["a1"], dout, 1, 1, nm["w_proj"], x_scale=B["gate"])
        se = nm["se"]
        groups = 0
        if 16 <= hw <= 256:
            _, groups = self._conv_bwd_data(dout, w[nm["w_proj"]], 1, out=da2, ws=ws, gate=B["a1"], part=P.gate_part, out_block=out_block)
        else:
            self._conv_bwd_data(dout, w[nm["w_proj"]], 1, out=da2, ws=ws)
        se_outs = dict(dpre1=B["dpre1"], dpre2=B["dpre2"], chan_add=B["chan_add"])
        if not groups and bn1_sums:
            nbs = ops.se_bn_bwd_sums(B["z1"], da2, *S.bn_bwd_args(B["st1"], nm["bn1"]), P.sums_part)
            ops.se_mlp_bwd_bn(P.sums_part, nbs, B["gate"], B["hpre"], w[se[0]], w[se[2]], hw, se_outs, P.stage1_se, w1t=self.wt[se[0]])
            return tgt_has or b.skip, (P.stage1_se, N)
        if not groups:
            if out_block:
                raise MliisError("internal: the project backward-data launch of block {} left no gate-gradient partials for its "
                                 "group-blocked output".format(b.idx))
            ops.colsum(da2, B["a1"], nseg=N, out=B["dgate"], ws=ws)
        ops.se_mlp_bwd(P.gate_part if groups else B["dgate"], B["gate"], B["s"], B["hpre"], w[se[0]], w[se[2]], hw, se_outs,
                       dgate_groups=groups, w1t=self.wt[se[0]])
        return tgt_has or b.skip, None

    def _mbconv_expand_bwd(self, S: _Pass, bi, B, nm, da0, tgt, tgt_has):
        P, w = S.P, S.w
        S.wgrad_conv(B["x_in"], da0, 1, 1, nm["w_exp"])
        if bi == 0:
            self._conv_bwd_data(da0, w[nm["w_exp"]], 1, out=tgt, accumulate=tgt_has, ws=S.ws)
            return None
        Bp = P.blocks[bi - 1]
        _, nb = self._conv_bwd_data(da0, w[nm["w_exp"]], 1, out=tgt, accumulate=tgt_has, ws=S.ws,
                                    bn=(Bp["z2"], Bp["st2"][0], Bp["st2"][1], Bp["dc"] if Bp["use_dc"] else None), part=P.stats_part)
        return (P.stats_part, nb) if nb else None

    def _mbconv_small_bwd(self, S: _Pass, bi, b, B, nm, tgt, tgt_has, stage1):
        w, g, p0, p1, da0 = S.w, S.g, nm["bn0"], nm["bn1"], B["da0"]
        tgt_has, _ = self._mbconv_project_bwd(S, b, B, nm, tgt, tgt_has, stage1, out_block=B["blk"], bn1_sums=False)
        ops.mbconv_dw_bwd_small(B["da2"], B["gate"], B["chan_add"], B["z1"], S.bn_bwd_args(B["st1"], p1), w[nm["w_dw"]], B["z0"],
                                S.bn_bwd_args(B["st0"], p0), g[p1 + "/gamma"], g[p1 + "/beta"], g[nm["w_dw"]], g[p0 + "/gamma"], g[p0 + "/beta"],
                                da0, z0_blocked=B["z0b"], z1_blocked=True, da2_blocked=bool(B["blk"]))
        return self._mbconv_expand_bwd(S, bi, B, nm, da0, tgt, tgt_has)

    def _mbconv_march_bwd(self, S: _Pass, bi, b, B, nm, tgt, tgt_has, stage1):
        P, w, g, da2 = S.P, S.w, S.g, B["da2"]
        tgt_has, bn1_stage1 = self._mbconv_project_bwd(S, b, B, nm, tgt, tgt_has, stage1)
        wdw, slabs = w[nm["w_dw"]], P.fold_part[nm["w_dw"]]
        if b.expand != 1:
            zin, st0, p0, dxo = B["z0"], B["st0"], nm["bn0"], B["da0"]
        elif bi == 0 and P.fuse_stem:
            zin, st0, p0, dxo = P.z_stem, P.st_stem, self.n_stem[1], tgt
        else:
            zin = None
        fuse_bn1 = bn1_stage1 is not None and not (b.k == 5 and b.stride == 1) and zin is not None
        if not fuse_bn1:
            S.bn_b(B["z1"], da2, B["st1"], nm["bn1"], da2, post=True, chan_scale=B["gate"], chan_add=B["chan_add"], stage1=bn1_stage1)
        if zin is None:
            S.noexpand_dw_bwd(B, tgt, tgt_has, lambda out: ops.dwconv_bn_bwd(da2, B["x_in"], wdw, b.stride, out=out, dw_part=slabs))
            return None
        if fuse_bn1:
            p1, ce, N = nm["bn1"], b.cexp, P.N
            nb1 = ops.mbconv_dw_bwd_march(da2, B["z1"], S.bn_bwd_args(B["st1"], p1), B["gate"], B["chan_add"],
                                          P.stage1_se[:2 * N * ce].view(N, 2, ce), g[p1 + "/gamma"], g[p1 + "/beta"], zin,
                                          S.bn_bwd_args(st0, p0), wdw, b.stride, dxo, slabs, P.stats_part2)
        else:
            _, _, nb1 = ops.dwconv_bn_bwd(da2, zin, wdw, b.stride, bn=S.bn_bwd_args(st0, p0), out=dxo, dw_part=slabs, bn_part=P.stats_part2)
        if b.expand == 1:
            return P.stats_part2, nb1
        S.bn_b(B["z0"], dxo, st0, p0, dxo, post=True, stage1=(P.stats_part2, nb1))
        return self._mbconv_expand_bwd(S, bi, B, nm, dxo, tgt, tgt_has)

    def _mbconv_opbyop_bwd(self, S: _Pass, bi, b, B, nm, tgt, tgt_has, stage1):
        P, w, da2 = S.P, S.w, B["da2"]
        tgt_has, bn1_stage1 = self._mbconv_project_bwd(S, b, B, nm, tgt, tgt_has, stage1)
        S.bn_b(B["z1"], da2, B["st1"], nm["bn1"], da2, post=True, chan_scale=B["gate"], chan_add=B["chan_add"], stage1=bn1_stage1)
        ops.dwconv_bwd_filter(B["a0"] if b.expand != 1 else B["x_in"], da2, b.k, b.stride, partial=P.fold_part[nm["w_dw"]])
        if b.expand == 1:
            S.noexpand_dw_bwd(B, tgt, tgt_has, lambda out: ops.dwconv_bwd_data(da2, w[nm["w_dw"]], b.stride, (b.h_in, b.h_in), out=out))
            return None
        da0, st0 = B["da0"], B["st0"]
        _, nb1 = ops.dwconv_bwd_data(da2, w[nm["w_dw"]], b.stride, (b.h_in, b.h_in), out=da0, part=P.stats_part,
                                     bn=(B["z0"],) + S.bn_bwd_args(st0, nm["bn0"]))
        S.bn_b(B["z0"], da0, st0, nm["bn0"], da0, post=True, stage1=(P.stats_part, nb1) if nb1 else None)
        return self._mbconv_expand_bwd(S, bi, B, nm, da0, tgt, tgt_has)

    def _stem_bwd(self, S: _Pass, x, idx, stage1):
        P = S.P
        S.bn_b(P.z_stem, P.dstem, P.st_stem, self.n_stem[1], P.dstem, post=True, stage1=stage1)
        ops.stem_conv_bwd_filter(x, P.dstem, idx, partial=P.fold_part[self.n_stem[0]])
```

Measured before the change: 3587.

## Use channel-pair lanes for fp32 depthwise-march backward kernels and fuse k5 s1 BN1

Templates the depthwise march conv kernels on a vector width, so fp32 backward variants can run with float2 channel pairs and 512-thread blocks instead of float4 quads and 256 threads. This halves per-thread register state (the K*K filter-gradient accumulators), aiming at better occupancy and latency hiding. For K=5 with the fused BN1 path, it parks per-channel constants in shared memory to cut register pressure. It also enables the fused BN1 backward for k=5 stride-1 blocks that previously ran a separate bn_b pass. The cost is more block-level reduction traffic and narrower memory accesses.

After: 3621, median of 6. Within noise of the previous version (+1.0%).

```diff
diff --git a/mliis_amd/csrc/dwmarch.hip b/mliis_amd/csrc/dwmarch.hip
--- a/mliis_amd/csrc/dwmarch.hip
+++ b/mliis_amd/csrc/dwmarch.hip
@@ -1,3 +1,5 @@
+#include <type_traits>
+
 #include "bn_fold.hpp"
 #include "common.hpp"
 
@@ -40,6 +42,45 @@
 }
 __device__ __forceinline__ float4 f4sel(bool ok, const float4 v) { return ok ? v : make_float4(0.f, 0.f, 0.f, 0.f); }
 template <typename T> __device__ __forceinline__ float4 dwm_stored(const float4 v) { return stored_value(static_cast<const T*>(nullptr), v); }
+
+__device__ __forceinline__ float vget(const float4& v, int i) { return i == 0 ? v.x : i == 1 ? v.y : i == 2 ? v.z : v.w; }
+__device__ __forceinline__ float vget(const float2& v, int i) { return i == 0 ? v.x : v.y; }
+template <typename VT, typename F>
+__device__ __forceinline__ VT vmap(F f) {
+  if constexpr (sizeof(VT) == 16) return make_float4(f(0), f(1), f(2), f(3));
+  else return make_float2(f(0), f(1));
+}
+template <typename VT> __device__ __forceinline__ VT vzero() { return vmap<VT>([](int) { return 0.f; }); }
+template <typename VT> __device__ __forceinline__ VT vadd(const VT a, const VT b) { return vmap<VT>([&](int i) { return vget(a, i) + vget(b, i); }); }
+template <typename VT> __device__ __forceinline__ VT vmul(const VT a, const VT b) { return vmap<VT>([&](int i) { return vget(a, i) * vget(b, i); }); }
+template <typename VT> __device__ __forceinline__ VT vfma(const VT a, const VT b, const VT c) {
+  return vmap<VT>([&](int i) { return fmaf(vget(a, i), vget(b, i), vget(c, i)); });
+}
+template <typename VT> __device__ __forceinline__ VT vsel(bool ok, const VT v) { return ok ? v : vzero<VT>(); }
+template <typename VT> __device__ __forceinline__ VT vld(const float* p) { return *reinterpret_cast<const VT*>(p); }
+template <typename VT> __device__ __forceinline__ void vst(float* p, const VT v) { *reinterpret_cast<VT*>(p) = v; }
+template <typename T, typename VT>
+__device__ __forceinline__ VT dwm_ldv(__amdgpu_buffer_rsrc_t r, int off, bool ok) {
+  if constexpr (sizeof(VT) == 16) {
+    return dwm_load<T>(r, off, ok);
+  } else {
+    static_assert(sizeof(T) == 4, "channel pairs: fp32 storage");
+    const dwm_u32x2 u = __builtin_amdgcn_raw_buffer_load_b64(r, ok ? off : (int)kDwmOob, 0, 0);
+    return make_float2(__uint_as_float(u.x), __uint_as_float(u.y));
+  }
+}
+template <typename T, typename VT>
+__device__ __forceinline__ void dwm_stv(__amdgpu_buffer_rsrc_t r, int off, bool ok, const VT v) {
+  if constexpr (sizeof(VT) == 16) {
+    dwm_store<T>(r, off, ok, v);
+  } else {
+    static_assert(sizeof(T) == 4, "channel pairs: fp32 storage");
+    dwm_u32x2 u;
+    u.x = __float_as_uint(v.x); u.y = __float_as_uint(v.y);
+    __builtin_amdgcn_raw_buffer_store_b64(u, r, ok ? off : (int)kDwmOob, 0, kDwmStoreAux);
+  }
+}
+template <typename T> __device__ __forceinline__ float2 dwm_stored(const float2 v) { return v; }
 
 template <int K, int S>
 struct MarchCfg {
@@ -72,41 +113,48 @@
   double inv_rows;
   float *dgamma, *dbeta;
 };
-struct DwmDyQuad {
-  float4 sc, sh, gt, ca, k1, k0;
+template <typename VT>
+struct DwmDyQuadT {
+  VT sc, sh, gt, ca, k1, k0;
 };
-__device__ __forceinline__ DwmDyQuad dwm_dybn_setup(const DwmDyBn& d, int C, int c0, int q, bool cok, int n, bool lead) {
-  const int c = cok ? c0 + q * 4 : 0;
-  const float4 m = ld4(d.mean + c), rs = ld4(d.rstd + c), ga = ld4(d.gamma + c), be = ld4(d.beta + c);
-  DwmDyQuad k;
-  k.gt = ld4(d.gate + (long long)n * C + c);
-  k.ca = ld4(d.chan_add + (long long)n * C + c);
-  double s1[4] = {0, 0, 0, 0}, s2[4] = {0, 0, 0, 0};
+template <typename VT>
+__device__ __forceinline__ DwmDyQuadT<VT> dwm_dybn_setup(const DwmDyBn& d, int C, int c, int n, bool publish) {
+  constexpr int V = (int)sizeof(VT) / 4;
+  const VT m = vld<VT>(d.mean + c), rs = vld<VT>(d.rstd + c), ga = vld<VT>(d.gamma + c), be = vld<VT>(d.beta + c);
+  DwmDyQuadT<VT> k;
+  k.gt = vld<VT>(d.gate + (long long)n * C + c);
+  k.ca = vld<VT>(d.chan_add + (long long)n * C + c);
+  double s1[V], s2[V];
+#pragma unroll
+  for (int e = 0; e < V; ++e) s1[e] = s2[e] = 0.0;
   for (int i0 = 0; i0 < d.nimg; i0 += 8) {
-    float4 u[8], v[8];
+    VT u[8], v[8];
 #pragma unroll
     for (int j = 0; j < 8; ++j) {
       const int i = i0 + j < d.nimg ? i0 + j : d.nimg - 1;
-      u[j] = ld4(d.stage1 + ((long long)i * 2 + 0) * C + c);
-      v[j] = ld4(d.stage1 + ((long long)i * 2 + 1) * C + c);
+      u[j] = vld<VT>(d.stage1 + ((long long)i * 2 + 0) * C + c);
+      v[j] = vld<VT>(d.stage1 + ((long long)i * 2 + 1) * C + c);
     }
 #pragma unroll
     for (int j = 0; j < 8; ++j)
       if (i0 + j < d.nimg) {
-        s1[0] += u[j].x; s1[1] += u[j].y; s1[2] += u[j].z; s1[3] += u[j].w;
-        s2[0] += v[j].x; s2[1] += v[j].y; s2[2] += v[j].z; s2[3] += v[j].w;
+#pragma unroll
+        for (int e = 0; e < V; ++e) {
+          s1[e] += vget(u[j], e);
+          s2[e] += vget(v[j], e);
+        }
       }
   }
-  if (lead && cok && (threadIdx.x >> 3) == 0) {
-    st4(d.dbeta + c, make_float4((float)s1[0], (float)s1[1], (float)s1[2], (float)s1[3]));
-    st4(d.dgamma + c, make_float4((float)s2[0], (float)s2[1], (float)s2[2], (float)s2[3]));
-  }
-  const float4 a = make_float4((float)(s1[0] * d.inv_rows), (float)(s1[1] * d.inv_rows), (float)(s1[2] * d.inv_rows), (float)(s1[3] * d.inv_rows));
-  const float4 b = make_float4((float)(s2[0] * d.inv_rows), (float)(s2[1] * d.inv_rows), (float)(s2[2] * d.inv_rows), (float)(s2[3] * d.inv_rows));
-  k.sc = f4mul(ga, rs);
-  k.sh = make_float4(fmaf(-m.x, k.sc.x, be.x), fmaf(-m.y, k.sc.y, be.y), fmaf(-m.z, k.sc.z, be.z), fmaf(-m.w, k.sc.w, be.w));
-  k.k1 = make_float4(-k.sc.x * b.x * rs.x, -k.sc.y * b.y * rs.y, -k.sc.z * b.z * rs.z, -k.sc.w * b.w * rs.w);
-  k.k0 = make_float4(-k.sc.x * a.x - k.k1.x * m.x, -k.sc.y * a.y - k.k1.y * m.y, -k.sc.z * a.z - k.k1.z * m.z, -k.sc.w * a.w - k.k1.w * m.w);
+  if (publish) {
+    vst<VT>(d.dbeta + c, vmap<VT>([&](int e) { return (float)s1[e]; }));
+    vst<VT>(d.dgamma + c, vmap<VT>([&](int e) { return (float)s2[e]; }));
+  }
+  const VT a = vmap<VT>([&](int e) { return (float)(s1[e] * d.inv_rows); });
+  const VT b = vmap<VT>([&](int e) { return (float)(s2[e] * d.inv_rows); });
+  k.sc = vmul(ga, rs);
+  k.sh = vmap<VT>([&](int e) { return fmaf(-vget(m, e), vget(k.sc, e), vget(be, e)); });
+  k.k1 = vmap<VT>([&](int e) { return -vget(k.sc, e) * vget(b, e) * vget(rs, e); });
+  k.k0 = vmap<VT>([&](int e) { return -vget(k.sc, e) * vget(a, e) - vget(k.k1, e) * vget(m, e); });
   return k;
 }
 __device__ __forceinline__ float dwm_dz1(float da2, float z, float sc, float sh, float gt, float ca, float k1, float k0) {
@@ -115,15 +163,17 @@
   const float g = fmaf(da2, gt, ca) * (sg * (1.0f + u * (1.0f - sg)));
   return fmaf(sc, g, fmaf(z, k1, k0));
 }
-__device__ __forceinline__ float4 dwm_dz1(const float4 da2, const float4 z, const DwmDyQuad& k) {
-  return make_float4(dwm_dz1(da2.x, z.x, k.sc.x, k.sh.x, k.gt.x, k.ca.x, k.k1.x, k.k0.x), dwm_dz1(da2.y, z.y, k.sc.y, k.sh.y, k.gt.y, k.ca.y, k.k1.y, k.k0.y),
-                     dwm_dz1(da2.z, z.z, k.sc.z, k.sh.z, k.gt.z, k.ca.z, k.k1.z, k.k0.z), dwm_dz1(da2.w, z.w, k.sc.w, k.sh.w, k.gt.w, k.ca.w, k.k1.w, k.k0.w));
-}
-
-template <int NEW, bool TWO>
+template <typename VT>
+__device__ __forceinline__ VT dwm_dz1(const VT da2, const VT z, const DwmDyQuadT<VT>& k) {
+  return vmap<VT>([&](int e) {
+    return dwm_dz1(vget(da2, e), vget(z, e), vget(k.sc, e), vget(k.sh, e), vget(k.gt, e), vget(k.ca, e), vget(k.k1, e), vget(k.k0, e));
+  });
+}
+
+template <int NEW, bool TWO, typename VT = float4>
 struct DwmBatch {
-  float4 a[NEW];
-  float4 b[TWO ? NEW : 1];
+  VT a[NEW];
+  VT b[TWO ? NEW : 1];
 };
 
 struct DwmArgs {
@@ -140,9 +190,38 @@
   float* dw_part;
 };
 
-struct DwmQuad {
-  float4 sc, sh, m, rs;
+template <typename VT>
+struct DwmQuadT {
+  VT sc, sh, m, rs;
 };
+typedef DwmQuadT<float4> DwmQuad;
+template <typename VT>
+struct DwmBnLoads {
+  VT g, b, m, rs;
+};
+template <typename VT>
+__device__ __forceinline__ DwmBnLoads<VT> dwm_bn_loads(const DwmBn& bn, int c) {
+  return DwmBnLoads<VT>{vld<VT>(bn.gamma + c), vld<VT>(bn.beta + c), vld<VT>(bn.f.mean + c), vld<VT>(bn.f.rstd + c)};
+}
+template <typename VT>
+__device__ __forceinline__ DwmQuadT<VT> dwm_bn_given(const DwmBnLoads<VT>& l) {
+  DwmQuadT<VT> k;
+  k.m = l.m;
+  k.rs = l.rs;
+  k.sc = vmul(l.g, l.rs);
+  k.sh = vmap<VT>([&](int e) { return fmaf(-vget(k.m, e), vget(k.sc, e), vget(l.b, e)); });
+  return k;
+}
+template <typename VT> __device__ __forceinline__ VT dwm_u(const VT z, const DwmQuadT<VT>& k) {
+  return vmap<VT>([&](int e) { return fmaf(vget(z, e), vget(k.sc, e), vget(k.sh, e)); });
+}
+template <typename VT> __device__ __forceinline__ VT dwm_sigmoid(const VT u) { return vmap<VT>([&](int e) { return sigmoid_f(vget(u, e)); }); }
+template <typename VT> __device__ __forceinline__ VT dwm_swish_bwd(const VT dy, const VT u, const VT sg) {
+  return vmap<VT>([&](int e) { return vget(dy, e) * vget(sg, e) * (1.0f + vget(u, e) * (1.0f - vget(sg, e))); });
+}
+template <typename VT> __device__ __forceinline__ VT dwm_xhat(const VT z, const DwmQuadT<VT>& k) {
+  return vmap<VT>([&](int e) { return (vget(z, e) - vget(k.m, e)) * vget(k.rs, e); });
+}
 
 __device__ __forceinline__ float4 dwm_act(const float4 z, const DwmQuad& k) {
   float4 u = make_float4(fmaf(z.x, k.sc.x, k.sh.x), fmaf(z.y, k.sc.y, k.sh.y), fmaf(z.z, k.sc.z, k.sh.z), fmaf(z.w, k.sc.w, k.sh.w));
@@ -215,51 +294,58 @@
   return k;
 }
 
-__device__ __forceinline__ void dwm_emit_pair(const float4 s1, const float4 s2, float4* buf, float* __restrict__ part, unsigned blk, int C,
-                                              int c0) {
-  const int t = threadIdx.x;
+template <typename VT>
+__device__ __forceinline__ void dwm_emit_pair(const VT s1, const VT s2, VT* buf, float* __restrict__ part, unsigned blk, int C, int c0) {
+  constexpr int V = (int)sizeof(VT) / 4, QL = 32 / V, NT = 32 * QL;
+  int t = threadIdx.x;
+  if (V == 2) asm volatile("" : "+v"(t));
   buf[t] = s1;
-  buf[256 + t] = s2;
+  buf[NT + t] = s2;
   __syncthreads();
-  float4 v = f4zero();
-  if (t < 64) {
-    const int qq = t & 7, g = (t >> 3) & 3, vv = t >> 5;
-#pragma unroll
-    for (int i = 0; i < 8; ++i) v = f4add(v, buf[vv * 256 + (g * 8 + i) * 8 + qq]);
+  VT v = vzero<VT>();
+  if (t < 8 * QL) {
+    const int qq = t % QL, g = (t / QL) & 3, vv = t / (4 * QL);
+#pragma unroll
+    for (int i = 0; i < 8; ++i) v = vadd(v, buf[vv * NT + (g * 8 + i) * QL + qq]);
   }
   __syncthreads();
-  if (t < 64) buf[t] = v;
+  if (t < 8 * QL) buf[t] = v;
   __syncthreads();
-  if (t < 16) {
-    const int qq = t & 7, vv = t >> 3;
-    const int cc = c0 + qq * 4;
-    const float4* b4 = buf + vv * 32 + qq;
-    if (cc < C) st4(part + ((long long)blk * 2 + vv) * C + cc, f4add(f4add(b4[0], b4[8]), f4add(b4[16], b4[24])));
-  }
-}
-
-template <int K, int S, bool PRE, bool BWD, bool DYBN = false, typename TA = float, typename TB = float>
-__global__ __launch_bounds__(256, BWD ? 1 : 2) void dwm_conv_k(const DwmArgs a) {
+  if (t < 2 * QL) {
+    const int qq = t % QL, vv = t / QL;
+    const int cc = c0 + qq * V;
+    const VT* b4 = buf + vv * 4 * QL + qq;
+    if (cc < C) vst<VT>(part + ((long long)blk * 2 + vv) * C + cc, vadd(vadd(b4[0], b4[QL]), vadd(b4[2 * QL], b4[3 * QL])));
+  }
+}
+
+template <int K, int S, bool PRE, bool BWD, bool DYBN = false, typename TA = float, typename TB = float, int V = 4>
+__global__ __launch_bounds__(32 * (32 / V), (BWD && V == 4) ? 1 : (V == 4 ? 2 : 1)) void dwm_conv_k(const DwmArgs a) {
   constexpr int EA = (int)sizeof(TA), EB = (int)sizeof(TB);
+  constexpr int QL = 32 / V, NT = 32 * QL, NW = NT / 64;
+  typedef typename std::conditional<V == 4, float4, float2>::type VT;
+  static_assert(V == 4 || (V == 2 && BWD), "channel pairs are a backward form");
   static_assert(!DYBN || BWD, "DYBN is a backward mode");
   typedef MarchCfg<K, S> G;
   constexpr int TS = G::TS, SPR = G::SPR, RS = G::RS, IBW = G::IBW, IBWP = G::IBWP, WIN = G::WIN, NEW = G::NEW, NR = G::NR, WW = G::WW;
   static_assert(!BWD || S == 1, "the stride-2 backward is dwm_bwd_s2_k");
-  constexpr int kRingF4 = (NR * IBWP + 1) * 8;
-  constexpr int kTrash = NR * IBWP * 8;
-  constexpr int kScratchF4 = BWD ? (K * K * 4 * 8) : 0;
+  constexpr int kRingF4 = (NR * IBWP + 1) * QL;
+  constexpr int kTrash = NR * IBWP * QL;
+  constexpr int kScratchF4 = BWD ? (K * K * NW * QL) : 0;
   constexpr int kSharedF4 = kRingF4 > kScratchF4 ? kRingF4 : kScratchF4;
-  static_assert(kSharedF4 * 16 >= 2 * 32 * 32 * 8, "the statistics fold borrows the ring");
-  __shared__ float4 ring[kSharedF4];
-  __shared__ float4 wl[K * K * 8];
+  static_assert(kSharedF4 * sizeof(VT) >= 2 * 32 * 32 * 8, "the statistics fold borrows the ring");
+  __shared__ VT ring[kSharedF4];
+  __shared__ VT wl[K * K * QL];
   __shared__ __attribute__((aligned(16))) float s_mr[64];
-
-  const int t = threadIdx.x, q = t & 7, p = t >> 3;
+  constexpr bool PARK = BWD && K == 5 && V == 2;
+  __shared__ VT s_kc[PARK ? 10 * QL : 1];
+
+  const int t = threadIdx.x, q = t % QL, p = t / QL;
   const unsigned bx = xcd_remap(blockIdx.x, gridDim.x);
   const int chunk = (int)(bx % (unsigned)a.chunks);
   const unsigned r_ = bx / (unsigned)a.chunks;
   const int band = (int)(r_ % (unsigned)a.bands), n = (int)(r_ / (unsigned)a.bands);
-  const int c0 = blockIdx.y * 32, c = c0 + q * 4;
+  const int c0 = blockIdx.y * 32, c = c0 + q * V;
   const bool cok = c < a.C;
   const int Hi = a.Hi, Wi = a.Wi, Ho = a.Ho, Wo = a.Wo, C = a.C;
   const int oy0 = chunk * a.rpc;
@@ -277,28 +363,37 @@
   const bool colok = cok && p < ibw && (unsigned)(ix0 + p) < (unsigned)Wi;
   const int tbase = (((n * Hi + iy0) * Wi + ix0 + p) * C + c) * EA;
   const int rowbytes = Wi * C * EA;
-  const int lcol = p < IBWP ? (p ^ ((p >> 2) & 1)) * 8 + q : kTrash + q;
+  const int lcol = p < IBWP ? (p ^ ((p >> 2) & 1)) * QL + q : kTrash + q;
   auto row_in = [&](int rr) { return rr >= 0 && rr < rows_needed && (unsigned)(iy0 + rr) < (unsigned)Hi; };
-  typedef DwmBatch<NEW, DYBN> Batch;
+  typedef DwmBatch<NEW, DYBN, VT> Batch;
   const __amdgpu_buffer_rsrc_t rX2 = dwm_rsrc(DYBN ? a.dyb.z : a.x);
   auto issue = [&](Batch& r, int rb) {
 #pragma unroll
     for (int j = 0; j < NEW; ++j) {
-      r.a[j] = dwm_load<TA>(rX, tbase + (rb + j) * rowbytes, colok && row_in(rb + j));
-      if (DYBN) r.b[j] = dwm_load<TA>(rX2, tbase + (rb + j) * rowbytes, colok && row_in(rb + j));
+      r.a[j] = dwm_ldv<TA, VT>(rX, tbase + (rb + j) * rowbytes, colok && row_in(rb + j));
+      if (DYBN) r.b[j] = dwm_ldv<TA, VT>(rX2, tbase + (rb + j) * rowbytes, colok && row_in(rb + j));
     }
   };
-  DwmQuad kq;
-  DwmDyQuad dq;
-  auto commit = [&](const Batch& r, int rb, int sb) {
+  DwmQuadT<VT> kq;
+  DwmDyQuadT<VT> dq;
+  auto parked = [&]() {
+    int o = q;
+    asm volatile("" : "+v"(o));
+    return s_kc + o;
+  };
+  auto commit = [&](const Batch& r, int rb, int sb, bool head) {
+    if (PARK && DYBN && !head) {
+      const VT* kc = parked();
+      dq.sc = kc[4 * QL]; dq.sh = kc[5 * QL]; dq.gt = kc[6 * QL]; dq.ca = kc[7 * QL]; dq.k1 = kc[8 * QL]; dq.k0 = kc[9 * QL];
+    }
 #pragma unroll
     for (int j = 0; j < NEW; ++j) {
-      float4 v = r.a[j];
-      if (PRE && !BWD) v = f4sel(colok && row_in(rb + j), dwm_act(v, kq));
-      if (DYBN) v = f4sel(colok && row_in(rb + j), dwm_dz1(v, r.b[j], dq));
+      VT v = r.a[j];
+      if constexpr (PRE && !BWD) v = f4sel(colok && row_in(rb + j), dwm_act(v, kq));
+      if constexpr (DYBN) v = vsel(colok && row_in(rb + j), dwm_dz1(v, r.b[j], dq));
       int slot = sb + j;
       if (slot >= NR) slot -= NR;
-      if (rb + j >= 0) ring[(p < IBWP ? slot * (IBWP * 8) : 0) + lcol] = v;
+      if (rb + j >= 0) ring[(p < IBWP ? slot * (IBWP * QL) : 0) + lcol] = v;
     }
   };
 
@@ -307,118 +402,128 @@
   const int colbase = sx < SPR ? sx * (TS * S) : 0;
   const int sxpar = sx & 1;
   const int zbase = BWD ? (((n * Ho + oy0 + ro) * Wo + ox0 + sx * TS) * C + c) * EB : 0;
-  auto issue_z = [&](float4 (&zr)[TS], int step) {
+  auto issue_z = [&](VT (&zr)[TS], int step) {
     if (BWD) {
       const int oy = oy0 + step * RS + ro;
       const int base = zbase + step * RS * Wo * C * EB;
 #pragma unroll
-      for (int u = 0; u < TS; ++u) zr[u] = dwm_load<TB>(rZ, base + u * C * EB, item_ok && oy < oy1 && sx * TS + u < bwa);
+      for (int u = 0; u < TS; ++u) zr[u] = dwm_ldv<TB, VT>(rZ, base + u * C * EB, item_ok && oy < oy1 && sx * TS + u < bwa);
     }
   };
 
   constexpr int HEAD = WIN - 2 * NEW;
-  float4 wreg = f4zero();
-  if (t < K * K * 8) {
-    const int tap = t >> 3, qq = t & 7;
-    const int cc = c0 + qq * 4;
-    if (cc < C) wreg = ld4(a.w + (long long)(BWD ? K * K - 1 - tap : tap) * C + cc);
+  VT wreg = vzero<VT>();
+  if (t < K * K * QL) {
+    const int tap = t / QL, qq = t % QL;
+    const int cc = c0 + qq * V;
+    if (cc < C) wreg = vld<VT>(a.w + (long long)(BWD ? K * K - 1 - tap : tap) * C + cc);
   }
   DwmBnState<!BWD> bst;
-  if (PRE) dwm_bn_begin(a.bn, C, c0, q, cok, bst);
-  if (DYBN) dq = dwm_dybn_setup(a.dyb, C, c0, q, cok, n, bx == 0);
+  DwmBnLoads<VT> bld;
+  if constexpr (PRE && BWD) bld = dwm_bn_loads<VT>(a.bn, cok ? c : 0);
+  if constexpr (PRE && !BWD) dwm_bn_begin(a.bn, C, c0, q, cok, bst);
+  if constexpr (DYBN) dq = dwm_dybn_setup<VT>(a.dyb, C, cok ? c : 0, n, bx == 0 && cok && p == 0);
   Batch ra, rb_;
-  float4 za[TS], zb[TS];
+  VT za[TS], zb[TS];
   {
     Batch h0, h1;
     issue(h0, HEAD);
     issue(h1, WIN - NEW);
     issue_z(za, 0);
-    if (PRE) kq = dwm_bn_end(a.bn, C, c0, q, cok, bx == 0, reinterpret_cast<double*>(ring), s_mr, bst);
+    if constexpr (PRE && BWD) kq = dwm_bn_given(bld);
+    if constexpr (PRE && !BWD) kq = dwm_bn_end(a.bn, C, c0, q, cok, bx == 0, reinterpret_cast<double*>(ring), s_mr, bst);
     issue(ra, WIN);
     issue(rb_, WIN + NEW);
     issue_z(zb, 1);
-    if (t < K * K * 8) wl[t] = wreg;
-    commit(h0, HEAD, HEAD < 0 ? HEAD + NR : HEAD);
-    commit(h1, WIN - NEW, (WIN - NEW) % NR);
+    if (t < K * K * QL) wl[t] = wreg;
+    commit(h0, HEAD, HEAD < 0 ? HEAD + NR : HEAD, true);
+    commit(h1, WIN - NEW, (WIN - NEW) % NR, true);
+    if (PARK && p == 0) {
+      if (PRE) { s_kc[q] = kq.sc; s_kc[QL + q] = kq.sh; s_kc[2 * QL + q] = kq.m; s_kc[3 * QL + q] = kq.rs; }
+      if (DYBN) {
+        s_kc[4 * QL + q] = dq.sc; s_kc[5 * QL + q] = dq.sh; s_kc[6 * QL + q] = dq.gt; s_kc[7 * QL + q] = dq.ca; s_kc[8 * QL + q] = dq.k1;
+        s_kc[9 * QL + q] = dq.k0;
+      }
+    }
   }
   __syncthreads();
 
-  float4 s1 = f4zero(), s2 = f4zero();
-  float4 dwacc[BWD ? K * K : 1];
+  VT s1 = vzero<VT>(), s2 = vzero<VT>();
+  VT dwacc[BWD ? K * K : 1];
   if (BWD) {
 #pragma unroll
-    for (int k = 0; k < K * K; ++k) dwacc[k] = f4zero();
+    for (int k = 0; k < K * K; ++k) dwacc[k] = vzero<VT>();
   }
 
   int sw = 0;
-  auto compute = [&](int step, const float4 (&zr)[TS]) {
+  auto compute = [&](int step, const VT (&zr)[TS]) {
     const int oy = oy0 + step * RS + ro;
     const bool row_ok = item_ok && oy < oy1;
     int s0 = sw + ro * S;
     if (s0 >= NR) s0 -= NR;
-    float4 acc[TS];
-#pragma unroll
-    for (int u = 0; u < TS; ++u) acc[u] = f4zero();
+    VT acc[TS];
+#pragma unroll
+    for (int u = 0; u < TS; ++u) acc[u] = vzero<VT>();
     int wofs = q;
     if (K == 5) asm volatile("" : "+v"(wofs));
-    const float4* wq = wl + wofs;
-    float4 av[TS], sgm[TS];
+    const VT* wq = wl + wofs;
+    VT av[TS], sgm[TS];
+    if (PARK && PRE) { const VT* kc = parked(); kq.sc = kc[0]; kq.sh = kc[QL]; }
     if (BWD) {
 #pragma unroll
       for (int u = 0; u < TS; ++u) {
         const bool ok = row_ok && sx * TS + u < bwa;
         if (PRE) {
-          const float4 z = zr[u];
-          const float4 uu = make_float4(fmaf(z.x, kq.sc.x, kq.sh.x), fmaf(z.y, kq.sc.y, kq.sh.y), fmaf(z.z, kq.sc.z, kq.sh.z), fmaf(z.w, kq.sc.w, kq.sh.w));
-          sgm[u] = f4sel(ok, make_float4(sigmoid_f(uu.x), sigmoid_f(uu.y), sigmoid_f(uu.z), sigmoid_f(uu.w)));
-          av[u] = f4mul(uu, sgm[u]);
+          const VT uu = dwm_u(zr[u], kq);
+          sgm[u] = vsel(ok, dwm_sigmoid(uu));
+          av[u] = vmul(uu, sgm[u]);
         } else {
-          av[u] = f4sel(ok, zr[u]);
+          av[u] = vsel(ok, zr[u]);
         }
       }
     }
-    auto read_row = [&](int ky, float4 (&in)[WW]) {
+    auto read_row = [&](int ky, VT (&in)[WW]) {
       int slot = s0 + ky;
       if (slot >= NR) slot -= NR;
       if constexpr ((TS * S) % 4 == 0) {
-        const float4* rowp = ring + slot * (IBWP * 8) + colbase * 8 + q;
-        const float4* A0 = rowp + sxpar * 8;
-        const float4* A1 = rowp - sxpar * 8;
+        const VT* rowp = ring + slot * (IBWP * QL) + colbase * QL + q;
+        const VT* A0 = rowp + sxpar * QL;
+        const VT* A1 = rowp - sxpar * QL;
 #pragma unroll
         for (int j = 0; j < WW; ++j) {
           const int je = j ^ ((j >> 2) & 1);
-          in[j] = ((je & 1) ? A1 : A0)[je * 8];
+          in[j] = ((je & 1) ? A1 : A0)[je * QL];
         }
       } else {
-        const float4* rowp = ring + slot * (IBWP * 8) + q;
+        const VT* rowp = ring + slot * (IBWP * QL) + q;
 #pragma unroll
         for (int j = 0; j < WW; ++j) {
           const int col = colbase + j;
-          in[j] = rowp[(col ^ ((col >> 2) & 1)) * 8];
+          in[j] = rowp[(col ^ ((col >> 2) & 1)) * QL];
         }
       }
     };
-    auto fma_row = [&](int ky, const float4 (&in)[WW]) {
-      float4 wk[K];
-#pragma unroll
-      for (int kx = 0; kx < K; ++kx) wk[kx] = wq[(ky * K + kx) * 8];
+    auto fma_row = [&](int ky, const VT (&in)[WW]) {
+      VT wk[K];
+#pragma unroll
+      for (int kx = 0; kx < K; ++kx) wk[kx] = wq[(ky * K + kx) * QL];
 #pragma unroll
       for (int kx = 0; kx < K; ++kx)
 #pragma unroll
         for (int u = 0; u < TS; ++u) {
-          acc[u] = f4fma(in[u * S + kx], wk[kx], acc[u]);
-          if (BWD) dwacc[ky * K + kx] = f4fma(in[u + kx], av[u], dwacc[ky * K + kx]);
+          acc[u] = vfma(in[u * S + kx], wk[kx], acc[u]);
+          if (BWD) dwacc[ky * K + kx] = vfma(in[u + kx], av[u], dwacc[ky * K + kx]);
         }
     };
     if (K == 3) {
-      float4 in[WW];
+      VT in[WW];
 #pragma unroll
       for (int ky = 0; ky < K; ++ky) {
         read_row(ky, in);
         fma_row(ky, in);
       }
     } else {
-      float4 inA[WW], inB[WW];
+      VT inA[WW], inB[WW];
       read_row(0, inA);
 #pragma unroll
       for (int ky = 0; ky < K; ++ky) {
@@ -428,24 +533,21 @@
       }
     }
     const int ybase = (((n * Ho + oy) * Wo + ox0 + sx * TS) * C + c) * EB;
+    if (PARK && PRE) { const VT* kc = parked(); kq.sc = kc[0]; kq.sh = kc[QL]; kq.m = kc[2 * QL]; kq.rs = kc[3 * QL]; }
     if (K == 5 && EB == 2) __builtin_amdgcn_sched_barrier(0);
 #pragma unroll
     for (int u = 0; u < TS; ++u) {
       const bool ok = row_ok && sx * TS + u < bwa;
       if (!(K == 5 && !BWD)) acc[u] = dwm_stored<TB>(acc[u]);
-      dwm_store<TB>(rY, ybase + u * C * EB, ok, acc[u]);
+      dwm_stv<TB, VT>(rY, ybase + u * C * EB, ok, acc[u]);
       if (!BWD) {
-        const float4 v = f4sel(ok, acc[u]);
-        s1 = f4add(s1, v);
-        s2 = f4fma(v, v, s2);
+        const VT v = vsel(ok, acc[u]);
+        s1 = vadd(s1, v);
+        s2 = vfma(v, v, s2);
       } else if (PRE) {
-        const float4 z = zr[u], sg_ = sgm[u];
-        const float4 uu = make_float4(fmaf(z.x, kq.sc.x, kq.sh.x), fmaf(z.y, kq.sc.y, kq.sh.y), fmaf(z.z, kq.sc.z, kq.sh.z), fmaf(z.w, kq.sc.w, kq.sh.w));
-        const float4 g = make_float4(acc[u].x * sg_.x * (1.0f + uu.x * (1.0f - sg_.x)), acc[u].y * sg_.y * (1.0f + uu.y * (1.0f - sg_.y)),
-                                     acc[u].z * sg_.z * (1.0f + uu.z * (1.0f - sg_.z)), acc[u].w * sg_.w * (1.0f + uu.w * (1.0f - sg_.w)));
-        const float4 xh = make_float4((z.x - kq.m.x) * kq.rs.x, (z.y - kq.m.y) * kq.rs.y, (z.z - kq.m.z) * kq.rs.z, (z.w - kq.m.w) * kq.rs.w);
-        s1 = f4add(s1, g);
-        s2 = f4fma(g, xh, s2);
+        const VT g = dwm_swish_bwd(acc[u], dwm_u(zr[u], kq), sgm[u]);
+        s1 = vadd(s1, g);
+        s2 = vfma(g, dwm_xhat(zr[u], kq), s2);
       }
     }
   };
@@ -454,14 +556,14 @@
   int sbn = WIN % NR;
   for (int i = 0; i < nsteps; i += 2) {
     compute(i, za);
-    commit(ra, rbn, sbn);
+    commit(ra, rbn, sbn, false);
     issue(ra, rbn + 2 * NEW);
     issue_z(za, i + 2);
     rbn += NEW; sbn += NEW; if (sbn >= NR) sbn -= NR;
     sw += NEW; if (sw >= NR) sw -= NR;
     __syncthreads();
     if (i + 1 < nsteps) compute(i + 1, zb);
-    commit(rb_, rbn, sbn);
+    commit(rb_, rbn, sbn, false);
     issue(rb_, rbn + 2 * NEW);
     issue_z(zb, i + 3);
     rbn += NEW; sbn += NEW; if (sbn >= NR) sbn -= NR;
@@ -472,47 +574,55 @@
   if (a.stats_part != nullptr && (!BWD || PRE)) dwm_emit_pair(s1, s2, ring, a.stats_part, bx, C, c0);
   if (BWD) {
     __syncthreads();
-    float4* fold = ring;
+    VT* fold = ring;
+    int te = t;
+    if (V == 2) asm volatile("" : "+v"(te));
 #pragma unroll
     for (int k = 0; k < K * K; ++k) {
-      float4 v = dwacc[k];
-#pragma unroll
-      for (int off = 8; off < 64; off <<= 1) {
-        v.x += __shfl_xor(v.x, off); v.y += __shfl_xor(v.y, off); v.z += __shfl_xor(v.z, off); v.w += __shfl_xor(v.w, off);
-      }
-      if ((t & 63) < 8) fold[(k * 4 + (t >> 6)) * 8 + q] = v;
+      VT v = dwacc[k];
+#pragma unroll
+      for (int off = QL; off < 64; off <<= 1) v = vmap<VT>([&](int e) { return vget(v, e) + __shfl_xor(vget(v, e), off); });
+      if ((te & 63) < QL) fold[(k * NW + (te >> 6)) * QL + te % QL] = v;
     }
     __syncthreads();
-    for (int e = t; e < K * K * 8; e += 256) {
-      const int k = e >> 3, qq = e & 7;
-      const int cc = c0 + qq * 4;
-      if (cc < C)
-        st4(a.dw_part + ((long long)bx * (K * K) + (K * K - 1 - k)) * C + cc,
-            f4add(f4add(fold[(k * 4 + 0) * 8 + qq], fold[(k * 4 + 1) * 8 + qq]), f4add(fold[(k * 4 + 2) * 8 + qq], fold[(k * 4 + 3) * 8 + qq])));
-    }
-  }
-}
-
-template <int K, bool PRE, bool DYBN = false, typename TA = float, typename TB = float>
-__global__ __launch_bounds__(256, (K == 5 || DYBN) ? 1 : 2) void dwm_bwd_s2_k(const DwmArgs a) {
+    for (int e = te; e < K * K * QL; e += NT) {
+      const int k = e / QL, qq = e % QL;
+      const int cc = c0 + qq * V;
+      VT f[NW];
+#pragma unroll
+      for (int w = 0; w < NW; ++w) f[w] = fold[(k * NW + w) * QL + qq];
+#pragma unroll
+      for (int w = NW; w > 1; w >>= 1)
+#pragma unroll
+        for (int i = 0; i < w / 2; ++i) f[i] = vadd(f[2 * i], f[2 * i + 1]);
+      if (cc < C) vst<VT>(a.dw_part + ((long long)bx * (K * K) + (K * K - 1 - k)) * C + cc, f[0]);
+    }
+  }
+}
+
+template <int K, bool PRE, bool DYBN = false, typename TA = float, typename TB = float, int V = 4>
+__global__ __launch_bounds__(32 * (32 / V), (V == 4 && !(K == 5 || DYBN)) ? 2 : 1) void dwm_bwd_s2_k(const DwmArgs a) {
   constexpr int EA = (int)sizeof(TA), EB = (int)sizeof(TB);
+  constexpr int QL = 32 / V, NT = 32 * QL, NW = NT / 64;
+  typedef typename std::conditional<V == 4, float4, float2>::type VT;
   constexpr int BP = 14;
   constexpr int D = (K - 1) / 2;
   constexpr int NEWD = 2, WIND = 2 + D, NR = WIND + NEWD, IBW = 16;
   static_assert(BP + D <= IBW, "one pixel lane per ring pixel of a batch");
-  constexpr int kRingF4 = NR * IBW * 8;
-  constexpr int kScratchF4 = K * K * 4 * 8;
-  constexpr int kSharedF4 = (kRingF4 > kScratchF4 ? kRingF4 : kScratchF4) > 1024 ? (kRingF4 > kScratchF4 ? kRingF4 : kScratchF4) : 1024;
-  __shared__ float4 ring[kSharedF4];
-  __shared__ float4 wl[K * K * 8];
+  constexpr int kRingF4 = NR * IBW * QL;
+  constexpr int kScratchF4 = K * K * NW * QL;
+  constexpr int kMinF4 = 16384 / (int)sizeof(VT);
+  constexpr int kSharedF4 = (kRingF4 > kScratchF4 ? kRingF4 : kScratchF4) > kMinF4 ? (kRingF4 > kScratchF4 ? kRingF4 : kScratchF4) : kMinF4;
+  __shared__ VT ring[kSharedF4];
+  __shared__ VT wl[K * K * QL];
   __shared__ __attribute__((aligned(16))) float s_mr[64];
 
-  const int t = threadIdx.x, q = t & 7, p = t >> 3;
+  const int t = threadIdx.x, q = t % QL, p = t / QL;
   const unsigned bx = xcd_remap(blockIdx.x, gridDim.x);
   const int chunk = (int)(bx % (unsigned)a.chunks);
   const unsigned r_ = bx / (unsigned)a.chunks;
   const int band = (int)(r_ % (unsigned)a.bands), n = (int)(r_ / (unsigned)a.bands);
-  const int c0 = blockIdx.y * 32, c = c0 + q * 4;
+  const int c0 = blockIdx.y * 32, c = c0 + q * V;
   const bool cok = c < a.C;
   const int Hd = a.Hi, Wd = a.Wi, H = a.Ho, W = a.Wo, C = a.C, pt = a.pt, pl = a.pl;
   const int my_lo = pt >> 1, my_hi = (H + pt - 1) >> 1;
@@ -531,20 +641,20 @@
   const bool colok = cok && scol < bpa + D && (unsigned)(x0 - D + scol) < (unsigned)Wd;
   const int tbase = (((n * Hd + m0 - D + sl) * Wd + x0 - D + scol) * C + c) * EA;
   const int rowbytes = Wd * C * EA;
-  typedef DwmBatch<1, DYBN> Batch;
+  typedef DwmBatch<1, DYBN, VT> Batch;
   const __amdgpu_buffer_rsrc_t rX2 = dwm_rsrc(DYBN ? a.dyb.z : a.x);
   auto row_in = [&](int rr) { return rr >= 0 && rr < rows_needed && (unsigned)(m0 - D + rr) < (unsigned)Hd; };
   auto issue = [&](Batch& r, int rb) {
-    r.a[0] = dwm_load<TA>(rX, tbase + rb * rowbytes, colok && row_in(rb + sl));
-    if (DYBN) r.b[0] = dwm_load<TA>(rX2, tbase + rb * rowbytes, colok && row_in(rb + sl));
+    r.a[0] = dwm_ldv<TA, VT>(rX, tbase + rb * rowbytes, colok && row_in(rb + sl));
+    if (DYBN) r.b[0] = dwm_ldv<TA, VT>(rX2, tbase + rb * rowbytes, colok && row_in(rb + sl));
   };
-  DwmDyQuad dq;
+  DwmDyQuadT<VT> dq;
   auto commit = [&](const Batch& r, int rb, int sb) {
     int slot = sb + sl;
     if (slot >= NR) slot -= NR;
-    float4 v = r.a[0];
-    if (DYBN) v = f4sel(colok && row_in(rb + sl), dwm_dz1(v, r.b[0], dq));
-    if (rb + sl >= 0) ring[slot * (IBW * 8) + scol * 8 + q] = v;
+    VT v = r.a[0];
+    if constexpr (DYBN) v = vsel(colok && row_in(rb + sl), dwm_dz1(v, r.b[0], dq));
+    if (rb + sl >= 0) ring[slot * (IBW * QL) + scol * QL + q] = v;
   };
 
   const int rp = p >> 4, px = p & 15;
@@ -559,70 +669,67 @@
     const int hi = 2 * (m0 + 2 * step + rp) + (u >> 1) - pt, wi = wi0 + (u & 1);
     return (((n * H + hi) * W + wi) * C + c) * EB;
   };
-  auto issue_z = [&](float4 (&zr)[4], int step) {
-#pragma unroll
-    for (int u = 0; u < 4; ++u) zr[u] = dwm_load<TB>(rZ, pix_off(step, u), pix_ok(step, u));
+  auto issue_z = [&](VT (&zr)[4], int step) {
+#pragma unroll
+    for (int u = 0; u < 4; ++u) zr[u] = dwm_ldv<TB, VT>(rZ, pix_off(step, u), pix_ok(step, u));
   };
 
   constexpr int HEAD = WIND - 2 * NEWD;
-  float4 wreg = f4zero();
-  if (t < K * K * 8) {
-    const int tap = t >> 3, qq = t & 7;
-    const int cc = c0 + qq * 4;
-    if (cc < C) wreg = ld4(a.w + (long long)tap * C + cc);
-  }
-  DwmQuad kq;
-  DwmBnState<false> bst;
-  if (PRE) dwm_bn_begin(a.bn, C, c0, q, cok, bst);
-  if (PRE) kq = dwm_bn_end(a.bn, C, c0, q, cok, false, reinterpret_cast<double*>(ring), s_mr, bst);
-  if (DYBN) dq = dwm_dybn_setup(a.dyb, C, c0, q, cok, n, bx == 0);
+  VT wreg = vzero<VT>();
+  if (t < K * K * QL) {
+    const int tap = t / QL, qq = t % QL;
+    const int cc = c0 + qq * V;
+    if (cc < C) wreg = vld<VT>(a.w + (long long)tap * C + cc);
+  }
+  DwmQuadT<VT> kq;
+  if constexpr (PRE) kq = dwm_bn_given(dwm_bn_loads<VT>(a.bn, cok ? c : 0));
+  if constexpr (DYBN) dq = dwm_dybn_setup<VT>(a.dyb, C, cok ? c : 0, n, bx == 0 && cok && p == 0);
   Batch ra, rb_, h0, h1;
-  float4 za[4], zb[4];
+  VT za[4], zb[4];
   issue(h0, HEAD);
   issue(h1, WIND - NEWD);
   issue_z(za, 0);
   issue(ra, WIND);
   issue(rb_, WIND + NEWD);
   issue_z(zb, 1);
-  if (t < K * K * 8) wl[t] = wreg;
+  if (t < K * K * QL) wl[t] = wreg;
   commit(h0, HEAD, HEAD < 0 ? HEAD + NR : HEAD);
   commit(h1, WIND - NEWD, (WIND - NEWD) % NR);
   __syncthreads();
 
-  float4 s1 = f4zero(), s2 = f4zero();
-  float4 dwacc[K * K];
-#pragma unroll
-  for (int k = 0; k < K * K; ++k) dwacc[k] = f4zero();
+  VT s1 = vzero<VT>(), s2 = vzero<VT>();
+  VT dwacc[K * K];
+#pragma unroll
+  for (int k = 0; k < K * K; ++k) dwacc[k] = vzero<VT>();
 
   int sw = 0;
-  auto compute = [&](int step, const float4 (&zr)[4]) {
-    float4 av[4], sgm[4], acc[4];
+  auto compute = [&](int step, const VT (&zr)[4]) {
+    VT av[4], sgm[4], acc[4];
 #pragma unroll
     for (int u = 0; u < 4; ++u) {
       const bool ok = pix_ok(step, u);
-      acc[u] = f4zero();
+      acc[u] = vzero<VT>();
       if (PRE) {
-        const float4 z = zr[u];
-        const float4 uu = make_float4(fmaf(z.x, kq.sc.x, kq.sh.x), fmaf(z.y, kq.sc.y, kq.sh.y), fmaf(z.z, kq.sc.z, kq.sh.z), fmaf(z.w, kq.sc.w, kq.sh.w));
-        sgm[u] = f4sel(ok, make_float4(sigmoid_f(uu.x), sigmoid_f(uu.y), sigmoid_f(uu.z), sigmoid_f(uu.w)));
-        av[u] = f4mul(uu, sgm[u]);
+        const VT uu = dwm_u(zr[u], kq);
+        sgm[u] = vsel(ok, dwm_sigmoid(uu));
+        av[u] = vmul(uu, sgm[u]);
       } else {
-        av[u] = f4sel(ok, zr[u]);
+        av[u] = vsel(ok, zr[u]);
       }
     }
     int s0 = sw + rp;
     if (s0 >= NR) s0 -= NR;
     int wofs = q;
     if (K == 5) asm volatile("" : "+v"(wofs));
-    const float4* wq = wl + wofs;
+    const VT* wq = wl + wofs;
 #pragma unroll
     for (int wr = 0; wr <= D; ++wr) {
       int slot = s0 + wr;
       if (slot >= NR) slot -= NR;
-      const float4* rowp = ring + slot * (IBW * 8) + pxc * 8 + q;
-      float4 dv[D + 1];
-#pragma unroll
-      for (int wc = 0; wc <= D; ++wc) dv[wc] = rowp[wc * 8];
+      const VT* rowp = ring + slot * (IBW * QL) + pxc * QL + q;
+      VT dv[D + 1];
+#pragma unroll
+      for (int wc = 0; wc <= D; ++wc) dv[wc] = rowp[wc * QL];
 #pragma unroll
       for (int pa = 0; pa < 2; ++pa) {
         const int ky = pa + 2 * (D - wr);
@@ -634,8 +741,8 @@
             const int kx = pb + 2 * (D - wc);
             if (kx > K - 1) continue;
             const int u = pa * 2 + pb, tap = ky * K + kx;
-            acc[u] = f4fma(dv[wc], wq[tap * 8], acc[u]);
-            dwacc[tap] = f4fma(dv[wc], av[u], dwacc[tap]);
+            acc[u] = vfma(dv[wc], wq[tap * QL], acc[u]);
+            dwacc[tap] = vfma(dv[wc], av[u], dwacc[tap]);
           }
       }
       __builtin_amdgcn_sched_barrier(0);
@@ -643,15 +750,11 @@
 #pragma unroll
     for (int u = 0; u < 4; ++u) {
       acc[u] = dwm_stored<TB>(acc[u]);
-      dwm_store<TB>(rY, pix_off(step, u), pix_ok(step, u), acc[u]);
+      dwm_stv<TB, VT>(rY, pix_off(step, u), pix_ok(step, u), acc[u]);
       if (PRE) {
-        const float4 z = zr[u], sg_ = sgm[u];
-        const float4 uu = make_float4(fmaf(z.x, kq.sc.x, kq.sh.x), fmaf(z.y, kq.sc.y, kq.sh.y), fmaf(z.z, kq.sc.z, kq.sh.z), fmaf(z.w, kq.sc.w, kq.sh.w));
-        const float4 g = make_float4(acc[u].x * sg_.x * (1.0f + uu.x * (1.0f - sg_.x)), acc[u].y * sg_.y * (1.0f + uu.y * (1.0f - sg_.y)),
-                                     acc[u].z * sg_.z * (1.0f + uu.z * (1.0f - sg_.z)), acc[u].w * sg_.w * (1.0f + uu.w * (1.0f - sg_.w)));
-        const float4 xh = make_float4((z.x - kq.m.x) * kq.rs.x, (z.y - kq.m.y) * kq.rs.y, (z.z - kq.m.z) * kq.rs.z, (z.w - kq.m.w) * kq.rs.w);
-        s1 = f4add(s1, g);
-        s2 = f4fma(g, xh, s2);
+        const VT g = dwm_swish_bwd(acc[u], dwm_u(zr[u], kq), sgm[u]);
+        s1 = vadd(s1, g);
+        s2 = vfma(g, dwm_xhat(zr[u], kq), s2);
       }
     }
   };
@@ -676,23 +779,26 @@
 
   if (a.stats_part != nullptr && PRE) dwm_emit_pair(s1, s2, ring, a.stats_part, bx, C, c0);
   __syncthreads();
-  float4* fold = ring;
+  VT* fold = ring;
 #pragma unroll
   for (int k = 0; k < K * K; ++k) {
-    float4 v = dwacc[k];
-#pragma unroll
-    for (int off = 8; off < 64; off <<= 1) {
-      v.x += __shfl_xor(v.x, off); v.y += __shfl_xor(v.y, off); v.z += __shfl_xor(v.z, off); v.w += __shfl_xor(v.w, off);
-    }
-    if ((t & 63) < 8) fold[(k * 4 + (t >> 6)) * 8 + q] = v;
+    VT v = dwacc[k];
+#pragma unroll
+    for (int off = QL; off < 64; off <<= 1) v = vmap<VT>([&](int e) { return vget(v, e) + __shfl_xor(vget(v, e), off); });
+    if ((t & 63) < QL) fold[(k * NW + (t >> 6)) * QL + q] = v;
   }
   __syncthreads();
-  for (int e = t; e < K * K * 8; e += 256) {
-    const int k = e >> 3, qq = e & 7;
-    const int cc = c0 + qq * 4;
-    if (cc < C)
-      st4(a.dw_part + ((long long)bx * (K * K) + k) * C + cc,
-          f4add(f4add(fold[(k * 4 + 0) * 8 + qq], fold[(k * 4 + 1) * 8 + qq]), f4add(fold[(k * 4 + 2) * 8 + qq], fold[(k * 4 + 3) * 8 + qq])));
+  for (int e = t; e < K * K * QL; e += NT) {
+    const int k = e / QL, qq = e % QL;
+    const int cc = c0 + qq * V;
+    VT f[NW];
+#pragma unroll
+    for (int w = 0; w < NW; ++w) f[w] = fold[(k * NW + w) * QL + qq];
+#pragma unroll
+    for (int w = NW; w > 1; w >>= 1)
+#pragma unroll
+      for (int i = 0; i < w / 2; ++i) f[i] = vadd(f[2 * i], f[2 * i + 1]);
+    if (cc < C) vst<VT>(a.dw_part + ((long long)bx * (K * K) + k) * C + cc, f[0]);
   }
 }
 
@@ -784,9 +890,16 @@
   if (ta == MLIIS_DT_BF16 && tb == MLIIS_DT_BF16) return true;
   return bwd ? (ta == MLIIS_DT_BF16 && tb == MLIIS_DT_F32) : (ta == MLIIS_DT_F32 && tb == MLIIS_DT_BF16);
 }
+constexpr bool dwm_pairs(int K, int S) { return K == 5 || S == 1; }
 template <int K, int S, bool PRE, bool BWD>
 static void launch_conv(const MarchGeom& g, const DwmArgs& a, int ta, int tb, hipStream_t stream) {
   const dim3 grid((unsigned)g.gx, g.gy);
+  if constexpr (BWD && dwm_pairs(K, S)) {
+    if (ta == MLIIS_DT_F32 && tb == MLIIS_DT_F32) {
+      hipLaunchKernelGGL((dwm_conv_k<K, S, PRE, BWD, false, float, float, 2>), grid, dim3(512), 0, stream, a);
+      return;
+    }
+  }
   if (ta == MLIIS_DT_F32 && tb == MLIIS_DT_F32) hipLaunchKernelGGL((dwm_conv_k<K, S, PRE, BWD, false, float, float>), grid, dim3(256), 0, stream, a);
   else if (ta == MLIIS_DT_BF16 && tb == MLIIS_DT_BF16) hipLaunchKernelGGL((dwm_conv_k<K, S, PRE, BWD, false, bf16s, bf16s>), grid, dim3(256), 0, stream, a);
   else if constexpr (BWD) hipLaunchKernelGGL((dwm_conv_k<K, S, PRE, BWD, false, bf16s, float>), grid, dim3(256), 0, stream, a);
@@ -795,15 +908,18 @@
 template <int K, bool PRE>
 static void launch_bwd_s2(const MarchGeom& g, const DwmArgs& a, int ta, int tb, hipStream_t stream) {
   const dim3 grid((unsigned)g.gx, g.gy);
-  if (ta == MLIIS_DT_F32) hipLaunchKernelGGL((dwm_bwd_s2_k<K, PRE, false, float, float>), grid, dim3(256), 0, stream, a);
+  constexpr int V = dwm_pairs(K, 2) ? 2 : 4;
+  if (ta == MLIIS_DT_F32) hipLaunchKernelGGL((dwm_bwd_s2_k<K, PRE, false, float, float, V>), grid, dim3(32 * (32 / V)), 0, stream, a);
   else if (tb == MLIIS_DT_BF16) hipLaunchKernelGGL((dwm_bwd_s2_k<K, PRE, false, bf16s, bf16s>), grid, dim3(256), 0, stream, a);
   else hipLaunchKernelGGL((dwm_bwd_s2_k<K, PRE, false, bf16s, float>), grid, dim3(256), 0, stream, a);
 }
 template <int K, typename TA, typename TB>
 static void launch_bwd_dybn_t(const MarchGeom& g, const DwmArgs& a, int stride, hipStream_t stream) {
   const dim3 grid((unsigned)g.gx, g.gy);
-  if (stride == 1) hipLaunchKernelGGL((dwm_conv_k<K, 1, true, true, true, TA, TB>), grid, dim3(256), 0, stream, a);
-  else hipLaunchKernelGGL((dwm_bwd_s2_k<K, true, true, TA, TB>), grid, dim3(256), 0, stream, a);
+  constexpr bool f32 = sizeof(TA) == 4 && sizeof(TB) == 4;
+  constexpr int V1 = f32 && dwm_pairs(K, 1) ? 2 : 4, V2 = f32 && dwm_pairs(K, 2) ? 2 : 4;
+  if (stride == 1) hipLaunchKernelGGL((dwm_conv_k<K, 1, true, true, true, TA, TB, V1>), grid, dim3(32 * (32 / V1)), 0, stream, a);
+  else hipLaunchKernelGGL((dwm_bwd_s2_k<K, true, true, TA, TB, V2>), grid, dim3(32 * (32 / V2)), 0, stream, a);
 }
 template <int K>
 static void launch_bwd_dybn(const MarchGeom& g, const DwmArgs& a, int stride, int ta, int tb, hipStream_t stream) {
diff --git a/mliis_amd/passes.py b/mliis_amd/passes.py
--- a/mliis_amd/passes.py
+++ b/mliis_amd/passes.py
@@ -485,7 +485,7 @@
             zin, st0, p0, dxo = P.z_stem, P.st_stem, self.n_stem[1], tgt
         else:
             zin = None
-        fuse_bn1 = bn1_stage1 is not None and not (b.k == 5 and b.stride == 1) and zin is not None
+        fuse_bn1 = bn1_stage1 is not None and zin is not None
         if not fuse_bn1:
             S.bn_b(B["z1"], da2, B["st1"], nm["bn1"], da2, post=True, chan_scale=B["gate"], chan_add=B["chan_add"], stage1=bn1_stage1)
         if zin is None:
```
